# NVIDIA/DeepLearningExamples

Hardware: AMD Instinct MI355X
Metric: training samples/sec (higher is better)
Workload: dtype bf16; 1 GPU; ResNet-50 v1.5 (PyTorch/Classification/ConvNets) synthetic ImageNet 224x224, label smoothing 0.1, SGD momentum 0.875 (BASELINE.json configs[1]); batch_per_gpu=256, global_batch=256, layout=NHWC, hip_graph=False, parallelism=single GPU

## Files before the change

### deeplearningexamples_amd/_cabi.py

```python
import ctypes
import os

import torch

_HERE = os.path.dirname(os.path.abspath(__file__))
LIB_PATH = os.environ.get("DLE_LIB_PATH") or os.path.join(_HERE, "lib", "libdle_mi355x.so")

F32, F16, BF16 = 0, 1, 2
ACT_NONE, ACT_RELU, ACT_GELU, ACT_RELU_BWD, ACT_ADD, ACT_GELU_BWD, ACT_TANH, ACT_TANH_BWD = 0, 1, 2, 3, 4, 5, 6, 7
ACT_ADD_MASKED, ACT_MUL, ACT_GELU_DAUX = 8, 9, 10

_DT = {torch.float32: F32, torch.float16: F16, torch.bfloat16: BF16}

c_void_p, c_int, c_i64, c_float = ctypes.c_void_p, ctypes.c_int, ctypes.c_int64, ctypes.c_float
c_u64 = ctypes.c_uint64

_SIGS = {
    "dle_last_error": (ctypes.c_char_p, []),
    "dle_abi_version": (c_int, []),
    "dle_device_check": (c_int, [c_int, ctypes.c_char_p, c_int]),
    "dle_dot_interact_out_width": (c_int, [c_int, c_int]),
    "dle_dot_interact_fwd": (c_int, [c_void_p, c_void_p, c_int, c_int, c_int, c_int, c_int, c_void_p]),
    "dle_dot_interact_bwd": (c_int, [c_void_p, c_void_p, c_void_p, c_void_p, c_int, c_int, c_int, c_int,
                                     c_int, c_void_p]),
    "dle_dot_interact_bwd_checked": (c_int, [c_void_p, c_void_p, c_void_p, c_void_p, c_int, c_int, c_int, c_int,
                                             c_int, c_void_p, c_void_p]),
    "dle_dlrm_gather_interact_try": (c_int, [c_void_p] * 6 + [c_i64, c_int, c_int, c_int, c_void_p]),
    "dle_emb_gather_fwd": (c_int, [c_void_p, c_void_p, c_void_p, c_void_p, c_void_p, c_i64, c_int, c_int,
                                   c_int, c_i64, c_void_p]),
    "dle_emb_offset_indices": (c_int, [c_void_p, c_void_p, c_void_p, c_void_p, c_i64, c_int, c_void_p]),
    "dle_emb_grad_values": (c_int, [c_void_p, c_void_p, c_void_p, c_i64, c_int, c_void_p]),
    "dle_emb_sparse_sgd": (c_int, [c_void_p, c_void_p, c_void_p, c_void_p, c_float, c_void_p, c_void_p,
                                   c_i64, c_int, c_int, c_i64, c_int, c_void_p]),
    "dle_emb_small_table_mask": (c_int, [c_void_p, c_int, c_int, c_void_p]),
    "dle_emb_sgd_dedup": (c_int, [c_void_p, c_void_p, c_void_p, c_void_p, c_void_p, c_void_p, c_void_p,
                                  c_void_p, c_float, c_void_p, c_void_p, c_i64, c_int, c_int, c_i64, c_int,
                                  c_void_p]),
    "dle_emb_sgd_dedup_ws": (c_int, [c_void_p, c_void_p, c_void_p, c_void_p, c_void_p, c_void_p, c_void_p,
                                     c_void_p, c_float, c_void_p, c_void_p, c_i64, c_int, c_int, c_i64, c_int,
                                     c_void_p, c_i64, c_void_p]),
    "dle_emb_onehot_workspace_bytes": (c_i64, [c_int, c_i64]),
    "dle_emb_sgd_workspace_bytes": (c_i64, [c_void_p, c_int, c_int, c_i64]),
    "dle_emb_onehot_try": (c_int, [c_void_p, c_void_p, c_void_p, c_void_p, c_float, c_void_p, c_void_p, c_void_p, c_void_p,
                                   c_void_p, c_int, c_i64, c_int, c_int, c_i64, c_int, c_void_p, c_i64, c_void_p]),
    "dle_emb_onehot_partials": (c_int, [c_void_p, c_void_p, c_void_p, c_void_p, c_void_p, c_void_p, c_int, c_i64, c_int, c_int,
                                        c_i64, c_int, c_void_p, c_i64, c_void_p, c_void_p]),
    "dle_emb_adam_workspace_bytes": (c_i64, [c_void_p, c_int, c_int, c_i64]),
    "dle_emb_adam_dedup_ws": (c_int, [c_void_p] * 9 + [c_float, c_void_p, c_void_p, c_void_p, c_float, c_float, c_float, c_i64,
                                      c_int, c_int, c_i64, c_int, c_void_p, c_i64, c_void_p]),
    "dle_cast_rows": (c_int, [c_void_p, c_void_p, c_i64, c_int, c_int, c_i64, c_i64, c_int, c_int, c_void_p]),
    "dle_bce_logits": (c_int, [c_void_p, c_void_p, c_void_p, c_void_p, c_void_p, c_i64, c_i64, c_int, c_void_p]),
    "dle_conv1x1_bnbwd_dgrad": (c_int, [c_void_p] * 16 + [c_i64, c_int, c_int, c_int, c_int, c_void_p]),
    "dle_conv1x1_bnbwd_groups": (c_int, [c_int]),
    "dle_conv1x1_bnbwd_dgrad_wgrad": (c_int, [c_void_p] * 15 + [c_i64, c_void_p, c_void_p, c_void_p, c_i64, c_int, c_int, c_int, c_int,
                                              c_void_p]),
    "dle_conv1x1_bnbwd_wgrad_workspace": (c_i64, [c_int, c_int]),
    "dle_gemm_expand_masked_bnred": (c_int, [c_void_p] * 10 + [c_i64, c_int, c_int, c_int, c_i64, c_i64, c_i64, c_int, c_int, c_void_p]),
    "dle_bn_bwd_finish": (c_int, [c_void_p, c_int, c_int, c_void_p, c_void_p, c_int, c_void_p]),
    "dle_gemm_colsum": (c_int, [c_void_p, c_void_p, c_void_p, c_void_p, c_void_p, c_int, c_int, c_int, c_i64, c_i64, c_i64, c_int,
                                c_int, c_int, c_void_p, c_i64, c_void_p]),
    "dle_head_bce_workspace_bytes": (c_i64, [c_i64, c_int]),
    "dle_head_bce_fwd_bwd": (c_int, [c_void_p, c_void_p, c_void_p, c_void_p, c_void_p, c_void_p, c_void_p, c_void_p, c_void_p,
                                     c_void_p, c_void_p, c_void_p, c_i64, c_i64, c_int, c_i64, c_i64, c_int, c_void_p]),
    "dle_amp_update_scale": (c_int, [c_void_p, c_void_p, c_void_p, c_void_p, c_float, c_float, c_int, c_int,
                                     c_void_p]),
    "dle_check_nonfinite": (c_int, [c_void_p, c_void_p, c_i64, c_int, c_void_p]),
    "dle_axpby_f32": (c_int, [c_void_p, c_void_p, c_void_p, c_float, c_float, c_i64, c_void_p]),
    "dle_act_bwd": (c_int, [c_void_p, c_void_p, c_void_p, c_i64, c_int, c_int, c_void_p]),
    "dle_relu_bwd": (c_int, [c_void_p, c_void_p, c_void_p, c_i64, c_int, c_i64, c_i64, c_i64, c_int, c_void_p]),
    "dle_gemm": (c_int, [c_void_p, c_void_p, c_void_p, c_void_p, c_void_p, c_void_p, c_int, c_int, c_int,
                         c_i64, c_i64, c_i64, c_int, c_int, c_int, c_int, c_int, c_int, c_int, c_float,
                         c_void_p, c_i64, c_void_p]),
    "dle_conv2d_fwd": (c_int, [c_void_p, c_void_p, c_void_p, c_void_p] + [c_int] * 12 + [c_void_p]),
    "dle_conv2d_fwd_affine": (c_int, [c_void_p] * 6 + [c_int] * 11 + [c_void_p]),
    "dle_conv3x3_affine_launch_count": (c_i64, []),
    "dle_conv2d_grouped_fwd_affine": (c_int, [c_void_p] * 5 + [c_int] * 9 + [c_void_p]),
    "dle_se_gate": (c_int, [c_void_p] * 6 + [c_int] * 5 + [c_void_p]),
    "dle_se_apply": (c_int, [c_void_p] * 4 + [c_i64, c_int, c_int, c_int, c_int, c_void_p]),
    "dle_dwconv2d_act_fwd": (c_int, [c_void_p] * 6 + [c_i64] + [c_int] * 9 + [c_void_p]),
    "dle_dwconv2d_pool_bands": (c_int, [c_int] * 5),
    "dle_se_gate_act": (c_int, [c_void_p, c_int, c_float] + [c_void_p] * 5 + [c_int] * 4 + [c_void_p]),
    "dle_silu_avgpool_fwd": (c_int, [c_void_p, c_void_p, c_int, c_int, c_int, c_int, c_void_p]),
    "dle_ssd_decode_fwd": (c_int, [c_void_p, c_void_p, c_int, c_void_p, c_void_p, c_void_p, c_int, c_int, c_int, c_float, c_float,
                                   c_int, c_void_p]),
    "dle_ssd_nms_fwd": (c_int, [c_void_p] * 5 + [c_int, c_int, c_int, c_float, c_float, c_int, c_void_p]),
    "dle_ssd_select_fwd": (c_int, [c_void_p] * 9 + [c_int] * 5 + [c_void_p]),
    "dle_conv2d_dgrad": (c_int, [c_void_p, c_void_p, c_void_p, c_void_p] + [c_int] * 10 + [c_void_p]),
    "dle_conv2d_wgrad": (c_int, [c_void_p, c_void_p, c_void_p] + [c_int] * 12 + [c_void_p, c_i64, c_void_p]),
    "dle_nchw_to_nhwc": (c_int, [c_void_p, c_void_p, c_i64, c_int, c_i64, c_int, c_int, c_void_p]),
    "dle_gemm_expand_add_up2": (c_int, [c_void_p, c_void_p, c_void_p, c_void_p, c_int, c_int, c_int, c_i64, c_i64, c_i64, c_i64, c_int,
                                        c_int, c_int, c_int, c_void_p]),
    "dle_conv1x1_bnload_groups": (c_int, [c_int, c_int, c_int]),
    "dle_conv1x1_bnload_fwd": (c_int, [c_void_p] * 11 + [c_i64, c_int, c_int, c_int, c_int, c_void_p]),
    "dle_bn_relu_maxpool_fwd": (c_int, [c_void_p] * 8 + [c_int, c_int, c_int, c_int, c_int, c_void_p]),
    "dle_wgrad1x1_workspace": (c_i64, []),
    "dle_wgrad1x1_mode": (c_int, [c_int]),
    "dle_wgrad1x1_workspace_for": (c_i64, [c_int, c_int, c_int]),
    "dle_gemm8_mode": (c_int, [c_int]),
    "dle_gemm8_min_items": (c_int, [c_int]),
    "dle_gemm8_launch_count": (c_i64, []),
    "dle_wgrad1x1_try": (c_int, [c_void_p, c_void_p, c_void_p, c_int, c_int, c_int, c_int, c_int, c_void_p, c_i64, c_void_p]),
    "dle_conv3x3_wgrad_workspace": (c_i64, []),
    "dle_conv3x3_wgrad_mode": (c_int, [c_int]),
    "dle_stem_conv7_groups": (c_int, [c_int, c_int]),
    "dle_stem_conv7_fwd": (c_int, [c_void_p, c_void_p, c_void_p, c_void_p, c_i64, c_int, c_int, c_int, c_int, c_void_p]),
    "dle_stem_conv7_wgrad_workspace": (c_i64, [c_int, c_int]),
    "dle_stem_conv7_wgrad": (c_int, [c_void_p, c_void_p, c_void_p, c_void_p, c_i64, c_int, c_int, c_int, c_int, c_int, c_void_p]),
    "dle_stem_pack_weight": (c_int, [c_void_p, c_void_p, c_int, c_void_p]),
    "dle_bn_workspace_bytes": (c_i64, [c_i64, c_int]),
    "dle_bn_fwd_stats": (c_int, [c_void_p, c_i64, c_int, c_float, c_float, c_void_p, c_void_p, c_void_p, c_void_p,
                                 c_void_p, c_i64, c_int, c_void_p]),
    "dle_conv2d_fwd_colstats": (c_int, [c_void_p, c_void_p, c_void_p] + [c_int] * 10 + [c_void_p, c_i64, c_void_p, c_void_p]),
    "dle_bn_stats_from_partials": (c_int, [c_void_p, c_int, c_i64, c_int, c_float, c_float, c_void_p, c_void_p, c_void_p,
                                           c_void_p, c_void_p, c_i64, c_void_p]),
    "dle_bn_fwd_apply": (c_int, [c_void_p] * 8 + [c_i64, c_int, c_int, c_int, c_void_p]),
    "dle_rccl_available": (c_int, []),
    "dle_rccl_unique_id": (c_int, [c_void_p]),
    "dle_rccl_init": (c_int, [c_void_p, c_int, c_int, c_void_p]),
    "dle_rccl_count": (c_int, [c_void_p]),
    "dle_rccl_destroy": (c_int, [c_void_p]),
    "dle_rccl_allreduce": (c_int, [c_void_p, c_void_p, c_i64, c_int, c_int, c_void_p]),
    "dle_rccl_broadcast": (c_int, [c_void_p, c_void_p, c_i64, c_int, c_void_p]),
    "dle_rccl_alltoallv": (c_int, [c_void_p, c_void_p, c_void_p, c_void_p, c_void_p, c_int, c_void_p]),
    "dle_gemm8_relu_bits_try": (c_int, [c_void_p] * 5 + [c_int, c_int, c_int, c_i64, c_i64, c_int, c_void_p]),
    "dle_gemm_colsum_bits": (c_int, [c_void_p] * 5 + [c_int, c_int, c_int, c_i64, c_i64, c_int, c_int, c_void_p, c_i64, c_void_p]),
    "dle_bn_bwd_reduce2": (c_int, [c_void_p] * 12 + [c_i64, c_int, c_void_p, c_i64, c_int, c_void_p]),
    "dle_bn_fwd_apply2": (c_int, [c_void_p] * 12 + [c_i64, c_int, c_int, c_void_p]),
    "dle_conv1x1_bnload_fwd2": (c_int, [c_void_p] * 15 + [c_i64, c_int, c_int, c_int, c_int, c_void_p]),
    "dle_bn_bwd_reduce": (c_int, [c_void_p] * 8 + [c_i64, c_int, c_int, c_void_p, c_i64, c_int, c_void_p]),
    "dle_bn_bwd_apply": (c_int, [c_void_p] * 11 + [c_i64, c_int, c_int, c_void_p]),
    "dle_maxpool_fwd": (c_int, [c_void_p, c_void_p, c_void_p] + [c_int] * 8 + [c_void_p]),
    "dle_maxpool_bwd": (c_int, [c_void_p, c_void_p, c_void_p] + [c_int] * 8 + [c_void_p]),
    "dle_pool_bn_bwd_workspace_bytes": (c_i64, [c_int] * 4),
    "dle_pool_bn_bwd": (c_int, [c_void_p] * 10 + [c_int] * 4 + [c_void_p, c_i64, c_int, c_void_p]),
    "dle_avgpool_fwd": (c_int, [c_void_p, c_void_p, c_i64, c_int, c_int, c_int, c_void_p]),
    "dle_avgpool_bwd": (c_int, [c_void_p, c_void_p, c_i64, c_int, c_int, c_int, c_void_p]),
    "dle_upsample_zero": (c_int, [c_void_p, c_void_p, c_i64, c_int, c_int, c_int, c_int, c_int, c_int, c_int, c_void_p]),
    "dle_softmax_xent": (c_int, [c_void_p, c_void_p, c_void_p, c_void_p, c_void_p, c_void_p, c_i64, c_int, c_i64,
                                 c_i64, c_float, c_i64, c_int, c_void_p]),
    "dle_gemm_batched": (c_int, [c_void_p, c_void_p, c_void_p, c_int, c_int, c_int, c_i64, c_i64, c_i64, c_int, c_int,
                                 c_int, c_int, c_float, c_int, c_int, c_i64, c_i64, c_i64, c_i64, c_i64, c_i64, c_void_p]),
    "dle_layernorm_fwd": (c_int, [c_void_p] * 8 + [c_i64, c_int, c_float, c_int, c_void_p]),
    "dle_layernorm_workspace_bytes": (c_i64, [c_int]),
    "dle_layernorm_bwd": (c_int, [c_void_p] * 8 + [c_i64, c_int, c_int, c_void_p, c_i64, c_int, c_void_p]),
    "dle_embed_sum": (c_int, [c_void_p] * 6 + [c_i64, c_int, c_int, c_int, c_void_p]),
    "dle_embed_sum_packed": (c_int, [c_void_p] * 7 + [c_i64, c_int, c_int, c_void_p]),
    "dle_embed_scatter_add": (c_int, [c_void_p, c_void_p, c_void_p, c_i64, c_int, c_int, c_void_p]),
    "dle_rows_select_sum": (c_int, [c_void_p, c_void_p, c_void_p, c_i64, c_int, c_int, c_int, c_void_p, c_i64, c_int,
                                    c_void_p]),
    "dle_rows_gather": (c_int, [c_void_p, c_void_p, c_void_p, c_i64, c_int, c_int, c_void_p]),
    "dle_rows_scatter": (c_int, [c_void_p, c_void_p, c_void_p, c_i64, c_int, c_int, c_int, c_void_p]),
    "dle_softmax_fwd": (c_int, [c_void_p, c_void_p, c_i64, c_int, c_int, c_float, c_int, c_void_p]),
    "dle_softmax_bwd": (c_int, [c_void_p, c_void_p, c_i64, c_int, c_float, c_int, c_void_p]),
    "dle_dropout_add_layernorm_bwd": (c_int, [c_void_p] * 6 + [c_float] + [c_void_p] * 5 + [c_i64, c_int, c_int, c_void_p, c_i64, c_int, c_void_p]),
    "dle_dropout_fwd": (c_int, [c_void_p, c_void_p, c_void_p, c_i64, c_float, c_u64, c_u64, c_void_p, c_int, c_void_p]),
    "dle_dropout_bwd": (c_int, [c_void_p, c_void_p, c_void_p, c_i64, c_float, c_int, c_void_p]),
    "dle_dropout_add_layernorm_fwd": (c_int, [c_void_p] * 9 + [c_i64, c_int, c_float, c_float, c_u64, c_u64, c_void_p, c_int, c_void_p]),
    "dle_softmax_dropout_fwd": (c_int, [c_void_p] * 4 + [c_i64, c_int, c_int, c_float, c_float, c_u64, c_u64, c_void_p, c_int, c_void_p]),
    "dle_softmax_dropout_bwd": (c_int, [c_void_p, c_void_p, c_void_p, c_i64, c_int, c_float, c_float, c_int, c_void_p]),
    "dle_u8_nchw_normalize_nhwc": (c_int, [c_void_p] * 4 + [c_i64, c_int, c_i64, c_int, c_int, c_void_p]),
    "dle_conv2d_dgrad_s2": (c_int, [c_void_p] * 3 + [c_int] * 5 + [c_void_p, c_i64, c_int, c_void_p]),
    "dle_attention_supported": (c_int, [c_int, c_int]),
    "dle_attention_stats_floats": (c_int, [c_int]),
    "dle_attention_fwd": (c_int, [c_void_p] * 5 + [c_int] * 4 + [c_float, c_float, c_u64, c_u64, c_void_p, c_int, c_void_p]),
    "dle_attention_bwd": (c_int, [c_void_p] * 6 + [c_int] * 4 + [c_float, c_float, c_u64, c_u64, c_void_p, c_int, c_void_p]),
    "dle_attention_bwd_keep": (c_int, [c_void_p] * 7 + [c_int] * 4 + [c_float, c_float, c_u64, c_u64, c_void_p, c_int, c_void_p]),
    "dle_attention_varlen_supported": (c_int, [c_int, c_int]),
    "dle_attention_fwd_varlen": (c_int, [c_void_p] * 3 + [c_int, c_int, c_i64, c_int, c_int, c_float, c_int, c_void_p]),
    "dle_attention_varlen_launch_count": (c_u64, []),
    "dle_colsum": (c_int, [c_void_p, c_void_p, c_i64, c_int, c_i64, c_int, c_int, c_void_p, c_i64, c_void_p]),
    "dle_colsum_batched_workspace_bytes": (c_i64, [c_int, c_i64, c_int]),
    "dle_colsum_batched": (c_int, [c_void_p, c_int, c_i64, c_int, c_i64, c_int, c_void_p, c_i64, c_void_p]),
    "dle_mt_table_len": (c_i64, [c_int, c_int]),
    "dle_mt_table_fill": (c_i64, [c_void_p, c_int, c_int, c_void_p, c_void_p, c_int]),
    "dle_mt_l2norm": (c_int, [c_void_p, c_int, c_i64, c_int, c_int, c_void_p, c_void_p, c_void_p, c_int,
                              c_void_p, c_void_p]),
    "dle_mt_lamb_stage1": (c_int, [c_void_p, c_int, c_i64, c_int, c_int, c_void_p, c_float, c_float, c_float,
                                   c_void_p, c_int, c_float, c_int, c_float, c_void_p, c_void_p, c_void_p,
                                   c_void_p]),
    "dle_mt_lamb_stage1_norms": (c_int, [c_void_p, c_int, c_i64, c_int, c_int, c_void_p, c_float, c_float, c_float,
                                         c_void_p, c_int, c_float, c_int, c_float, c_void_p, c_void_p, c_void_p,
                                         c_void_p, c_void_p, c_void_p, c_void_p]),
    "dle_mt_lamb_stage2": (c_int, [c_void_p, c_int, c_i64, c_int, c_int, c_int, c_void_p, c_void_p, c_void_p,
                                   c_void_p, c_float, c_int, c_void_p]),
    "dle_mt_sgd": (c_int, [c_void_p, c_int, c_i64, c_int, c_int, c_int, c_void_p, c_void_p, c_float, c_float,
                           c_float, c_float, c_int, c_int, c_void_p, c_int, c_void_p]),
    "dle_mt_adam": (c_int, [c_void_p, c_int, c_i64, c_int, c_void_p, c_void_p, c_float, c_float, c_float, c_float,
                            c_float, c_void_p, c_void_p, c_void_p, c_float, c_void_p]),
    "dle_mt_adam_copy": (c_int, [c_void_p, c_int, c_i64, c_int, c_int, c_void_p, c_void_p, c_float, c_float, c_float, c_float,
                                 c_void_p, c_void_p, c_void_p, c_void_p]),
    "dle_mt_ema": (c_int, [c_void_p, c_int, c_i64, c_int, c_void_p, c_float, c_float, c_void_p]),
    "dle_wg_taps": (c_int, [c_void_p, c_void_p] + [c_int] * 6 + [c_i64, c_int, c_void_p]),
    "dle_wg_taps_bwd": (c_int, [c_void_p, c_void_p, c_void_p] + [c_int] * 6 + [c_i64, c_i64, c_int, c_void_p]),
    "dle_wg_gate_fwd": (c_int, [c_void_p, c_void_p, c_i64, c_int, c_i64, c_int, c_void_p]),
    "dle_wg_gate_bwd": (c_int, [c_void_p, c_void_p, c_void_p, c_i64, c_int, c_i64, c_i64, c_int, c_void_p]),
    "dle_wg_invconv_fwd": (c_int, [c_void_p, c_void_p, c_void_p, c_void_p, c_i64, c_int, c_int, c_void_p]),
    "dle_wg_invconv_bwd_partials": (c_int, [c_i64]),
    "dle_wg_invconv_bwd": (c_int, [c_void_p] * 8 + [c_float, c_void_p, c_i64, c_int, c_void_p]),
    "dle_wg_logdet_inv": (c_int, [c_void_p, c_void_p, c_void_p, c_void_p, c_int, c_void_p]),
    "dle_wg_coupling_partials": (c_int, [c_i64]),
    "dle_wg_coupling_fwd": (c_int, [c_void_p, c_void_p, c_void_p, c_void_p, c_i64, c_int, c_void_p]),
    "dle_wg_coupling_bwd": (c_int, [c_void_p] * 6 + [c_float, c_i64, c_int, c_int, c_void_p]),
    "dle_wg_loss": (c_int, [c_void_p, c_void_p, c_int, c_void_p, c_int, c_float, c_i64, c_void_p, c_void_p, c_void_p]),
    "dle_wg_dz_init": (c_int, [c_void_p, c_void_p, c_void_p, c_float, c_i64, c_void_p]),
    "dle_wg_weight_norm_fwd": (c_int, [c_void_p, c_void_p, c_void_p] + [c_int] * 5 + [c_void_p]),
    "dle_wg_weight_norm_bwd": (c_int, [c_void_p] * 5 + [c_int] * 4 + [c_void_p]),
    "dle_wg_upsample_weight": (c_int, [c_void_p] * 4 + [c_int] * 4 + [c_void_p]),
    "dle_wg_upsample_weight_bwd": (c_int, [c_void_p, c_void_p, c_int, c_int, c_int, c_void_p]),
    "dle_wg_weight_norm_fwd_batched": (c_int, [c_void_p, c_int, c_i64, c_int, c_void_p]),
    "dle_wg_weight_norm_bwd_batched": (c_int, [c_void_p, c_int, c_i64, c_void_p]),
    "dle_wg_logdet_inv_batched": (c_int, [c_void_p, c_void_p, c_void_p, c_void_p, c_void_p, c_int, c_void_p]),
    "dle_wg_flow_inv": (c_int, [c_void_p] * 6 + [c_i64, c_int, c_int, c_int, c_float, c_int, c_int, c_void_p]),
    "dle_wg_flow_inv_first": (c_int, [c_void_p, c_void_p, c_void_p, c_i64, c_int, c_float, c_int, c_void_p]),
    "dle_t2_tanh_fwd": (c_int, [c_void_p, c_void_p, c_i64, c_int, c_void_p]),
    "dle_t2_lstm_fwd": (c_int, [c_void_p, c_i64, c_void_p, c_void_p, c_void_p, c_i64, c_void_p, c_i64, c_void_p, c_i64, c_void_p,
                                c_i64, c_float, c_void_p, c_void_p, c_i64, c_void_p, c_i64, c_int, c_int, c_int, c_void_p]),
    "dle_t2_lstm_bwd": (c_int, [c_void_p, c_i64, c_void_p, c_i64, c_void_p, c_i64, c_void_p, c_void_p, c_i64, c_void_p, c_void_p,
                                c_i64, c_void_p, c_void_p, c_i64, c_float, c_void_p, c_void_p, c_int, c_int, c_int, c_void_p]),
    "dle_t2_attention_fwd": (c_int, [c_void_p] * 10 + [c_i64, c_void_p, c_i64, c_void_p, c_i64, c_void_p] + [c_int] * 7 + [c_void_p]),
    "dle_t2_attention_bwd": (c_int, [c_void_p, c_i64, c_void_p, c_i64, c_void_p, c_i64] + [c_void_p] * 14 + [c_int, c_int, c_void_p, c_void_p] +
                             [c_int] * 5 + [c_void_p]),
    "dle_a2a_blocks": (c_int, [c_void_p, c_void_p, c_int, c_int, c_void_p, c_int, c_int, c_void_p]),
    "dle_t2_sum_steps": (c_int, [c_void_p, c_void_p, c_int, c_i64, c_int, c_void_p]),
    "dle_t2_location_bwd": (c_int, [c_void_p, c_void_p, c_void_p, c_int, c_int, c_int, c_int, c_void_p]),
    "dle_transpose_cast": (c_int, [c_void_p, c_void_p, c_int, c_int, c_i64, c_i64, c_int, c_int, c_void_p]),
    "dle_t2_mel_loss": (c_int, [c_void_p, c_i64, c_void_p, c_void_p, c_void_p, c_void_p, c_i64, c_void_p, c_void_p, c_void_p, c_i64,
                                c_int, c_int, c_void_p]),
    "dle_t2_lstm_gemm_fwd": (c_int, [c_void_p, c_i64, c_void_p, c_i64, c_void_p, c_void_p, c_void_p, c_void_p, c_void_p, c_i64, c_void_p,
                                     c_i64, c_void_p, c_i64, c_void_p, c_i64, c_void_p, c_i64, c_float, c_int, c_int, c_int, c_int,
                                     c_void_p]),
    "dle_t2_mask_rows": (c_int, [c_void_p, c_i64, c_int, c_void_p, c_i64, c_int, c_float, c_int, c_void_p]),
    "dle_t2_prenet_infer": (c_int, [c_void_p, c_void_p, c_void_p, c_void_p, c_i64, c_void_p, c_void_p, c_u64, c_void_p, c_int, c_int,
                                    c_int, c_int, c_void_p]),
    "dle_t2_frame_infer": (c_int, [c_void_p, c_i64, c_void_p, c_i64] + [c_void_p] * 7 + [c_int, c_float, c_int, c_i64, c_void_p,
                                   c_void_p, c_void_p, c_i64, c_u64, c_int, c_int, c_int, c_int, c_int, c_void_p]),
    "dle_conv1d_lrelu_fwd": (c_int, [c_void_p] * 6 + [c_int] * 6 + [c_float, c_float, c_int, c_void_p]),
    "dle_hfg_post_fwd": (c_int, [c_void_p] * 4 + [c_int] * 4 + [c_float, c_int, c_void_p]),
    "dle_conv1d_packed_fwd": (c_int, [c_void_p] * 6 + [c_int, c_int, c_i64, c_int, c_int, c_int, c_float, c_int, c_void_p]),
    "dle_fp_relu_layernorm_fwd": (c_int, [c_void_p] * 7 + [c_i64, c_int, c_int, c_float, c_int, c_void_p]),
    "dle_fp_embed": (c_int, [c_void_p] * 6 + [c_int, c_int, c_i64, c_int, c_int, c_int, c_int, c_void_p]),
    "dle_fp_scalar_conv_add": (c_int, [c_void_p] * 5 + [c_int, c_int, c_i64, c_int, c_int, c_int, c_void_p]),
    "dle_fp_durations": (c_int, [c_void_p, c_int] + [c_void_p] * 5 + [c_int, c_int, c_i64, c_float, c_float, c_int, c_void_p]),
    "dle_fp_expand": (c_int, [c_void_p] * 7 + [c_int, c_int, c_i64, c_int, c_i64, c_int, c_int, c_int, c_void_p]),
    "dle_fp_unpack_mel": (c_int, [c_void_p] * 4 + [c_int, c_i64, c_int, c_int, c_int, c_void_p]),
# ... 183 lines not shown
```

### deeplearningexamples_amd/convnets/engine.py

```python
import copy
import math
from typing import Optional

import numpy as np
import os

import torch
import torch.distributed as dist

from .. import functional as F
from .. import multi_tensor as mt
from ..utils.amp import GradScalerState
from ..utils.buckets import GradBuckets
from ..utils import comm
from .resnet import Deferred, ResNet50


def lr_cosine_policy(base_lr, warmup_length, epochs, end_lr=0.0):
    def fn(iteration, epoch):
        if epoch < warmup_length:
            return base_lr * (epoch + 1) / warmup_length
        e, es = epoch - warmup_length, epochs - warmup_length
        return end_lr + 0.5 * (1 + np.cos(np.pi * e / es)) * (base_lr - end_lr)
    return fn


def lr_step_policy(base_lr, steps, decay_factor, warmup_length):
    def fn(iteration, epoch):
        if epoch < warmup_length:
            return base_lr * (epoch + 1) / warmup_length
        lr = base_lr
        for s in steps:
            if epoch >= s:
                lr *= decay_factor
        return lr
    return fn


def lr_linear_policy(base_lr, warmup_length, epochs):
    def fn(iteration, epoch):
        if epoch < warmup_length:
            return base_lr * (epoch + 1) / warmup_length
        return base_lr * (1 - (epoch - warmup_length) / (epochs - warmup_length))
    return fn


class ResNetTrainer:
    def __init__(self, model: ResNet50, lr: float, momentum=0.875, weight_decay=3.0517578125e-05, nesterov=False,
                 label_smoothing=0.1, compute_dtype=torch.bfloat16, bn_weight_decay=False, static_loss_scale=1.0,
                 world_size=1, process_group=None, bucket_mb=25, grad_acc_steps=1, ema=None):
        self.model = model
        self.grad_acc_steps = max(1, int(grad_acc_steps))
        self.steps_since_update = 0
        self.flat_acc = None
        self.dev = model.fc.weight.device
        self.dtype = compute_dtype
        self.momentum, self.wd, self.nesterov, self.smoothing = momentum, weight_decay, nesterov, label_smoothing
        self.world, self.pg = world_size, process_group
        self.bn_weight_decay = bn_weight_decay
        if world_size > 1:
            comm.broadcast_parameters_(list(model.parameters()) + list(model.buffers()), 0, process_group)
        self.stem, self.blocks = model.units()
        self.scaler = GradScalerState(self.dev, enabled=compute_dtype == torch.float16, init_scale=static_loss_scale,
                                      growth_interval=int(1e9))
        self.lr = torch.full((1,), lr, dtype=torch.float32, device=self.dev)
        self.first_step = True
        self.steps_done = 0
        named = dict(model.named_parameters())
        order = ["fc.weight", "fc.bias"]
        for (u1, u2, u3, ud) in reversed(self.blocks):
            for u in ([u3, ud] if ud is not None else [u3]) + [u2, u1]:
                order += [u.name_conv + ".weight", u.name_bn + ".weight", u.name_bn + ".bias"]
        order += ["conv1.weight", "bn1.weight", "bn1.bias"]
        assert sorted(order) == sorted(named), "parameter bookkeeping out of sync with the module tree"
        self.names = order
        self.params = [named[n] for n in order]
        total = sum(p.numel() for p in self.params)
        self.flat_grad = torch.zeros(total, dtype=torch.float32, device=self.dev)
        self.flat_mom = torch.zeros(total, dtype=torch.float32, device=self.dev)
        self.gview, self.mview, self.offset = {}, {}, {}
        o = 0
        for n, p in zip(order, self.params):
            self.offset[n] = o
            self.gview[n] = self.flat_grad[o:o + p.numel()]
            self.mview[n] = self.flat_mom[o:o + p.numel()]
            o += p.numel()
        self.comm_stream = torch.cuda.Stream(device=self.dev) if world_size > 1 else None
        self.buckets = GradBuckets(self.flat_grad, [(n, p.numel()) for n, p in zip(order, self.params)], bucket_mb,
                                   process_group, self.comm_stream) if world_size > 1 else None
        self.w16 = {}
        units = [self.stem] + [u for blk in self.blocks for u in blk if u is not None]
        self.units = units
        for u in units:
            w = named[u.name_conv + ".weight"]
            ko, ci, r, s = w.shape
            cp = (ci + 7) // 8 * 8
            u.w16 = torch.zeros((ko, r, s, cp), dtype=compute_dtype, device=self.dev)
            self.w16[u.name_conv + ".weight"] = u.w16
            u.ggamma = self.gview[u.name_bn + ".weight"]
            u.gbeta = self.gview[u.name_bn + ".bias"]
            if cp == ci:
                u.gw = self.gview[u.name_conv + ".weight"].view(ko, r, s, ci)
            else:
                u.gw = torch.zeros((ko, r, s, cp), dtype=torch.float32, device=self.dev)
        self.wgrad_stream = torch.cuda.Stream(device=self.dev) if (self.dev.type == "cuda" and
                                                                   os.environ.get("DLE_RN50_WGRAD_STREAM", "1") != "0") else None
        self._wgrad_keepalive = []
        for u in units:
            u.wgrad_stream, u.keepalive = self.wgrad_stream, self._wgrad_keepalive
        self.branch_stream = torch.cuda.Stream(device=self.dev) if (self.dev.type == "cuda" and
                                                                    os.environ.get("DLE_RN50_BRANCH_STREAM", "1") != "0") else None
        self._branch_keep = []
        if self.buckets is not None:
            self.buckets.extra_streams += [st for st in (self.wgrad_stream, self.branch_stream) if st is not None]
        self.stem4 = os.environ.get("DLE_RN50_STEM4", "1") != "0"
        self.fuse_up2 = os.environ.get("DLE_RN50_FUSE_UP2", "1") != "0"
        self.fuse_bn = os.environ.get("DLE_RN50_FUSE_BN", "1") != "0"
        self.fuse_bnred = os.environ.get("DLE_RN50_FUSE_BNRED", "1") != "0"
        self.fuse_dsbn = os.environ.get("DLE_RN50_FUSE_DSBN", "1") != "0"
        self.fuse_dsred = os.environ.get("DLE_RN50_FUSE_DSRED", "1") != "0"
        self.fuse_pool_bwd = os.environ.get("DLE_RN50_FUSE_POOLBWD", "1") != "0"
        self.stem.w2 = torch.zeros((64, 7, 8, 4), dtype=compute_dtype, device=self.dev)
        self.stem.gw_flat = self.gview["conv1.weight"]
        self.fc_w16 = torch.empty(model.fc.weight.shape, dtype=compute_dtype, device=self.dev)
        self.w16["fc.weight"] = self.fc_w16
        self.refresh_working_copies()
        self._build_tables()
        self.ema = None if ema is None else float(ema)
        self.ema_model = None
        if self.ema is not None:
            self._build_ema()

    @staticmethod
    def _phys(p):
        if p.dim() == 4:
            return p.data.permute(0, 2, 3, 1).reshape(-1)
        return p.data.reshape(-1)

    def _refresh_copies(self, model, units, stem, fc_w16):
        for u in units:
            w = u.conv.weight
            ko, ci, r, s = w.shape
            F.cast_rows(self._phys(w).view(ko * r * s, ci), self.dtype, cols_out=u.w16.shape[-1],
                        out=u.w16.view(ko * r * s, -1))
        F.cast(model.fc.weight.data, self.dtype, out=fc_w16)
        F.stem_pack_weight(model.conv1.weight.data, self.dtype, out=stem.w2)

    def refresh_working_copies(self):
        self._refresh_copies(self.model, self.units, self.stem, self.fc_w16)

    def _stem_image(self, images):
        cp = 4 if (self.stem4 and images.shape[-1] <= 224) else 8
        if images.dtype == torch.uint8:
            if getattr(self, "_mean_std", None) is None:
                from .dataloaders import IMAGENET_MEAN, IMAGENET_STD
                self._mean_std = (torch.tensor(IMAGENET_MEAN, device=self.dev) * 255.0, torch.tensor(IMAGENET_STD, device=self.dev) * 255.0)
            return F.u8_nchw_normalize_nhwc(images, self._mean_std[0], self._mean_std[1], self.dtype, cp)
        return F.nchw_to_nhwc(images, self.dtype, cp)

    def _build_tables(self):
        named = dict(zip(self.names, self.params))
        decay_copy, decay_plain, nodecay = ([], [], [], []), ([], [], []), ([], [], [])
        for n, p in named.items():
            g, m, ph = self.gview[n], self.mview[n], self._phys(p)
            assert ph.data_ptr() == p.data_ptr(), "parameter %s is not dense in memory order" % n
            if "bn" in n and not self.bn_weight_decay:
                for lst, t in zip(nodecay, (g, ph, m)):
                    lst.append(t)
            elif n in self.w16 and self.w16[n].numel() == p.numel():
                for lst, t in zip(decay_copy, (g, ph, m, self.w16[n].view(-1))):
                    lst.append(t)
            else:
                for lst, t in zip(decay_plain, (g, ph, m)):
                    lst.append(t)
        self.t_decay_copy = mt.TensorTable(list(decay_copy))
        self.t_decay_plain = mt.TensorTable(list(decay_plain))
        self.t_nodecay = mt.TensorTable(list(nodecay))

    def set_lr(self, lr: float):
        self.lr.fill_(lr)

    @staticmethod
    def _ema_entries(model):
        return [(k, v) for k, v in model.state_dict().items() if not k.endswith("num_batches_tracked")]

    def _build_ema(self):
        self.ema_model = copy.deepcopy(self.model)
        xs, es = [], []
        for (k, x), (ke, e) in zip(self._ema_entries(self.model), self._ema_entries(self.ema_model)):
            assert k == ke and x.shape == e.shape and x.stride() == e.stride(), "EMA copy of %s lost the master's layout" % k
            assert x.dtype == torch.float32 and e.dtype == torch.float32, "EMA runs on the fp32 master state (%s)" % k
            px, pe = self._phys(x), self._phys(e)
            assert px.data_ptr() == x.data_ptr() and pe.data_ptr() == e.data_ptr(), "%s is not dense in memory order" % k
            xs.append(px)
            es.append(pe)
        self.t_ema = mt.TensorTable([xs, es], chunk=mt.streaming_chunk([xs]))
        self.ema_coef = torch.empty(2, dtype=torch.float32, device=self.dev)
        self._ema_coef_views = (self.ema_coef[0:1], self.ema_coef[1:2])
        self._ema_mu_t = None
        self.set_ema_step(None)
        self.ema_stem, self.ema_blocks = self.ema_model.units()
        self.ema_units = [self.ema_stem] + [u for blk in self.ema_blocks for u in blk if u is not None]
        for u, src in zip(self.ema_units, self.units):
            u.w16 = torch.zeros_like(src.w16)
        self.ema_stem.w2 = torch.zeros_like(self.stem.w2)
        self.ema_fc_w16 = torch.empty_like(self.fc_w16)
        self.ema_dirty = True

    def set_ema_step(self, step):
        if self.ema is None:
            raise ValueError("this trainer keeps no averaged model: construct it with ema=<decay>")
        mu_t = self.ema if step is None else min(self.ema, (1.0 + step) / (10 + step))
        if mu_t != self._ema_mu_t:
            self._ema_coef_views[0].fill_(mu_t)
            self._ema_coef_views[1].fill_(1.0 - mu_t)
            self._ema_mu_t = mu_t
        self.ema_dirty = True

    def mark_ema_dirty(self):
        self.ema_dirty = True

    def _ema_eval_state(self):
        if self.ema is None:
            raise ValueError("this trainer keeps no averaged model: construct it with ema=<decay>")
        if self.ema_dirty:
            self._refresh_copies(self.ema_model, self.ema_units, self.ema_stem, self.ema_fc_w16)
            self.ema_dirty = False
        return self.ema_model, self.ema_stem, self.ema_blocks, self.ema_fc_w16

    def set_side_streams(self, enabled):
        if not hasattr(self, "_streams_saved"):
            self._streams_saved = (self.wgrad_stream, self.branch_stream)
        torch.cuda.synchronize(self.dev)
        self.wgrad_stream, self.branch_stream = self._streams_saved if enabled else (None, None)
        for u in self.units:
            u.wgrad_stream = self.wgrad_stream

    def _maybe_reduce(self, finished_param_name):
        if self.buckets is not None and getattr(self, "_reduce_now", True):
            self.buckets.grad_ready(finished_param_name)

    def _input(self, images):
        if images.dim() == 4 and not images.is_contiguous():
            images = images.contiguous()
        return images

    def infer(self, images, ema=False):
        model, stem, blocks, fc_w16 = self._ema_eval_state() if ema else (self.model, self.stem, self.blocks, self.fc_w16)
        x = self._stem_image(self._input(images))
        h, _ = F.maxpool_fwd(stem.forward_eval(x))
        for (u1, u2, u3, ud) in blocks:
            res = ud.forward_eval(h) if ud is not None else h
            h = u3.forward_eval(u2.forward_eval(u1.forward_eval(h)), residual=res)
        pooled = F.avgpool_fwd(h)
        return F.gemm(pooled, fc_w16, pooled.shape[0], fc_w16.shape[0], fc_w16.shape[1], True, True,
                      out_dtype=torch.float32, bias=model.fc.bias.data)

    def eval_step(self, images, target, ema=False):
        logits = self.infer(images, ema=ema)
        loss, _ = F.softmax_xent(logits, target, smoothing=0.0)
        return loss, logits

    def forward(self, images):
        x = self._stem_image(self._input(images))
        d0 = self.stem.forward(x, defer=self.fuse_bn)
        if isinstance(d0, Deferred) and d0.t.shape[1] % 2 == 0 and d0.t.shape[2] % 2 == 0:
            m0, self._amax, mask0 = F.bn_relu_maxpool_fwd(d0.t, d0.mean, d0.rstd, self.stem.bn.weight.data, self.stem.bn.bias.data)
            d0._done(None, mask0)
            self._pool_in_hw = d0.t.shape[1:3]
        else:
            a0 = d0.materialize() if isinstance(d0, Deferred) else d0
            m0, self._amax = F.maxpool_fwd(a0)
            self._pool_in_hw = a0.shape[1:3]
        h = m0
        bs = self.branch_stream
        fuse = self.fuse_bn
        for (u1, u2, u3, ud) in self.blocks:
            o1 = u1.forward(h)
            hy = h.y if isinstance(h, Deferred) else h
            if ud is not None and bs is not None:
                cur = torch.cuda.current_stream()
                bs.wait_stream(cur)
                self._branch_keep.clear()
                with torch.cuda.stream(bs):
                    res = ud.forward(hy, defer=self.fuse_dsbn)
                o2 = u2.forward(o1, defer=fuse)
                cur.wait_stream(bs)
                self._branch_keep.append(res)
            else:
                res = ud.forward(hy, defer=self.fuse_dsbn) if ud is not None else hy
                o2 = u2.forward(o1, defer=fuse)
            h = u3.forward(o2, residual=res, defer=fuse)
        if isinstance(h, Deferred):
            h = h.materialize()
        self._feat_hw = h.shape[1:3]
        self._pooled = F.avgpool_fwd(h)
        n = self._pooled.shape[0]
        logits = F.gemm(self._pooled, self.fc_w16, n, self.fc_w16.shape[0], self.fc_w16.shape[1], True, True,
                        out_dtype=torch.float32, bias=self.model.fc.bias.data)
        return logits

    def backward(self, dlogits):
        n = dlogits.shape[0]
        fcw = self.fc_w16
        if self.buckets is not None:
            self.buckets.fired = 0
        F.gemm(dlogits, self._pooled, fcw.shape[0], fcw.shape[1], n, False, False,
               out=self.gview["fc.weight"].view(fcw.shape), splitk=F.pick_splitk(fcw.shape[0], fcw.shape[1], n))
        F.colsum(dlogits, out=self.gview["fc.bias"])
        self._maybe_reduce("fc.weight"); self._maybe_reduce("fc.bias")
        gp = F.gemm(dlogits, fcw, n, fcw.shape[1], fcw.shape[0], True, False)
        g = F.avgpool_bwd(gp, self._feat_hw)
        for blk in self.blocks:
            for u in blk:
                if u is not None:
                    u.reduce_done = False
        for bi in range(len(self.blocks) - 1, -1, -1):
            u1, u2, u3, ud = self.blocks[bi]
            mask3 = u3.relu_mask()
            if ud is not None and self.fuse_dsred and u3.saved is not None and ud.saved is not None and mask3 is not None \
                    and not u3.reduce_done and u3.saved[1].shape == ud.saved[1].shape:
                F.bn_bwd_reduce2(g, mask3, u3.saved[1], u3.saved[3], u3.saved[4], u3.ggamma, u3.gbeta,
                                 ud.saved[1], ud.saved[3], ud.saved[4], ud.ggamma, ud.gbeta)
                u3.reduce_done = ud.reduce_done = True
            bs = self.branch_stream if ud is not None else None
            if bs is not None:
                cur = torch.cuda.current_stream()
                bs.wait_stream(cur)
                self._branch_keep.clear()
                with torch.cuda.stream(bs):
                    gskip = ud.backward(g, dy_mask=mask3, compact_dx=self.fuse_up2)
                self._branch_keep.append((gskip, g))
            g3 = u3.backward(g, bnred=u2 if self.fuse_bnred else None)
            self._done(u3)
            if ud is not None and bs is None:
                gskip = ud.backward(g, dy_mask=mask3, compact_dx=self.fuse_up2)
            elif ud is None:
                gskip = (g, mask3)
            g2 = u2.backward(g3)
            self._done(u2)
            if bs is not None:
                cur.wait_stream(bs)
            if ud is not None:
                self._done(ud)
            prev3 = self.blocks[bi - 1][2] if (self.fuse_bnred and ud is None and bi > 0) else None
            g = u1.backward(g2, dx_addend=gskip, bnred=prev3)
            self._done(u1)
        if self.fuse_pool_bwd:
            self.stem.backward(None, need_dx=False, pooled=(g, self._amax))
        else:
            g = F.maxpool_bwd(g, self._amax, self._pool_in_hw)
            self.stem.backward(g, need_dx=False)
        gw = self.stem.gw
        ko, r, s, cp = gw.shape
        stem_generic = self.stem.saved_c != 4
        if self.wgrad_stream is not None:
            torch.cuda.current_stream().wait_stream(self.wgrad_stream)
            self._wgrad_keepalive.clear()
        self._branch_keep.clear()
        if stem_generic:
            F.copy_rows(gw.view(ko * r * s, cp)[:, :3], self.gview["conv1.weight"].view(ko * r * s, 3))
        self._done(self.stem)

    def _done(self, u):
        for suffix, nm in ((".weight", u.name_conv), (".weight", u.name_bn), (".bias", u.name_bn)):
            self._maybe_reduce(nm + suffix)

    def optimizer_step(self):
        sc = self.scaler
        skip = sc.found_inf if sc.enabled else None
        inv = sc.inv_scale if sc.enabled else None
        kw = dict(momentum=self.momentum, nesterov=self.nesterov, first_step=self.first_step, skip_flag=skip,
                  inv_scale=inv, has_momentum=self.momentum != 0)
        mt.sgd(self.t_decay_copy, self.lr, weight_decay=self.wd, model_copy=True, **kw)
        mt.sgd(self.t_decay_plain, self.lr, weight_decay=self.wd, **kw)
        mt.sgd(self.t_nodecay, self.lr, weight_decay=0.0, **kw)
        u = self.stem
        w = self.model.conv1.weight
        F.stem_pack_weight(w.data, self.dtype, out=u.w2)
        ko, ci, r, s = w.shape
        F.cast_rows(self._phys(w).view(ko * r * s, ci), self.dtype, cols_out=u.w16.shape[-1], out=u.w16.view(ko * r * s, -1))
        self.first_step = False

    def train_step(self, images, target, step=None):
        loss = self._train_step(images, target)
        if self.ema is not None:
            if step is not None:
                self.set_ema_step(step)
            mt.ema(self.t_ema, self.ema, coef=self.ema_coef)
            self.ema_dirty = True
        return loss

    def _train_step(self, images, target):
        sc = self.scaler
        acc = self.grad_acc_steps
        self.steps_since_update += 1
        last = self.steps_since_update == acc
        logits = self.forward(images)
        gs = sc.scale if sc.enabled else None
        if isinstance(target, tuple):
            ya, yb, lam = target
            la, da = F.softmax_xent(logits, ya, smoothing=self.smoothing, grad_scale=gs, grad_dtype=torch.float32)
            lb, db = F.softmax_xent(logits, yb, smoothing=self.smoothing, grad_scale=gs, grad_dtype=torch.float32)
            loss = lam * la + (1.0 - lam) * lb
            F.axpby_(da.view(-1), db.view(-1), da.view(-1), lam, 1.0 - lam)
            dlogits = F.cast(da, self.dtype)
        else:
            loss, dlogits = F.softmax_xent(logits, target, smoothing=self.smoothing, grad_scale=gs, grad_dtype=self.dtype)
        self._reduce_now = acc == 1
        self.backward(dlogits)
        if acc > 1:
            if self.flat_acc is None:
                self.flat_acc = torch.empty_like(self.flat_grad)
            first = self.steps_since_update == 1
            dst = self.flat_grad if last else self.flat_acc
            F.axpby_(self.flat_grad, None if first else self.flat_acc, dst, 1.0 / acc, 0.0 if first else 1.0)
            loss = loss / acc
            if not last:
                self.steps_done += 1
                return loss
            if self.world > 1:
                comm.allreduce_mean_(self.flat_grad, self.pg)
        elif self.buckets is not None:
            self.buckets.wait()
        if sc.enabled:
            F.check_nonfinite_(self.flat_grad, sc.found_inf)
        self.optimizer_step()
        sc.update()
        self.steps_since_update = 0
        self.steps_done += 1
        return loss

    def reduced_loss(self, loss):
        if self.world > 1:
            loss = comm.allreduce_mean_(loss.clone(), self.pg)
        return loss

    def sync_counters(self):
        for u in self.units:
            u.bn.num_batches_tracked.fill_(self.steps_done)
```

### deeplearningexamples_amd/convnets/resnet.py

```python
from contextlib import nullcontext as _nullcontext
from typing import List

import os

import torch
from torch import nn

from .. import _cabi as C
from .. import functional as F

LAYERS, WIDTHS, EXPANSION = [3, 4, 6, 3], [64, 128, 256, 512], 4


def _conv(cin, cout, k, stride, device):
    m = nn.Conv2d(cin, cout, kernel_size=k, stride=stride, padding=(k - 1) // 2, bias=False, device=device)
    nn.init.kaiming_normal_(m.weight, mode="fan_in", nonlinearity="relu")
    m.weight.data = m.weight.data.contiguous(memory_format=torch.channels_last)
    return m


def _bn(c, device, zero_init=False):
    m = nn.BatchNorm2d(c, device=device)
    nn.init.constant_(m.weight, 0 if zero_init else 1)
    nn.init.constant_(m.bias, 0)
# ... 10 lines not shown
        r = self.residual
        if isinstance(r, Deferred):
            return r.t, (r.mean, r.rstd, r.unit.bn.weight.data, r.unit.bn.bias.data)
        return r, None

    def _done(self, y, mask):
        u = self.unit
        u.saved = (u.saved[0], self.t, mask, self.mean, self.rstd)
        self.y = y

    def materialize(self):
        if self.y is None:
            u = self.unit
            res, res_bn = self.residual_args()
            y, mask = F.bn_fwd_apply(self.t, self.mean, self.rstd, u.bn.weight.data, u.bn.bias.data, residual=res,
                                     relu=u.relu, want_mask=True, residual_bn=res_bn)
            self._done(y, mask)
        return self.y


class ConvBN:

    def __init__(self, conv: nn.Conv2d, bn: nn.BatchNorm2d, name_conv: str, name_bn: str, relu: bool):
        self.conv, self.bn, self.name_conv, self.name_bn, self.relu = conv, bn, name_conv, name_bn, relu
        self.k = conv.kernel_size[0]
        self.stride, self.pad = conv.stride[0], conv.padding[0]
        self.cin, self.cout = conv.in_channels, conv.out_channels
        self.w16 = None
        self.gw = self.ggamma = self.gbeta = None
        self.saved = None
        self.w2 = self.gw_flat = None
        self.wgrad_stream = None
        self.fuse_bnbwd = os.environ.get("DLE_RN50_FUSE_BNBWD", "1") != "0"
        self.fuse_bnbwd_wgrad = os.environ.get("DLE_RN50_FUSE_BNBWD_WGRAD", "1") != "0"
        self.reduce_done = False
        self.keepalive = None

    def forward(self, x, residual=None, defer=False):
        t = None
        if isinstance(x, Deferred):
            d, r = x, None
            if self.k == 1 and self.stride == 1 and d.unit.relu and d.y is None:
                res, res_bn = d.residual_args()
                r = F.conv1x1_bnload_fwd(d.t, res, self.w16, d.mean, d.rstd, d.unit.bn.weight.data, d.unit.bn.bias.data,
                                         self.bn.running_mean, self.bn.running_var, eps=self.bn.eps, momentum=self.bn.momentum,
                                         res_bn=res_bn)
            if r is not None:
                t, x, bits, mean, rstd = r
                d._done(x, bits)
            else:
                x = d.materialize()
        if t is None:
            if x.shape[-1] == 4:
                t, mean, rstd = F.stem_conv_fwd_bnstats(x, self.w2, self.bn.running_mean, self.bn.running_var, eps=self.bn.eps,
                                                        momentum=self.bn.momentum)
            else:
                t, mean, rstd = F.conv2d_fwd_bnstats(x, self.w16, self.stride, self.pad, self.bn.running_mean,
                                                     self.bn.running_var, eps=self.bn.eps, momentum=self.bn.momentum)
        if defer:
            self.saved = (x, t, None, mean, rstd)
            return Deferred(self, t, mean, rstd, residual)
        if isinstance(residual, Deferred):
            d = Deferred(self, t, mean, rstd, residual)
            self.saved = (x, t, None, mean, rstd)
            return d.materialize()
        y, mask = F.bn_fwd_apply(t, mean, rstd, self.bn.weight.data, self.bn.bias.data, residual=residual,
                                 relu=self.relu, want_mask=True)
        self.saved = (x, t, mask, mean, rstd)
        return y

    def forward_eval(self, x, residual=None):
        t = F.stem_conv_fwd(x, self.w2, want_stats=False)[0] if x.shape[-1] == 4 else F.conv2d_fwd(x, self.w16, self.stride, self.pad)
        rstd = torch.rsqrt(self.bn.running_var + self.bn.eps)
        y, _ = F.bn_fwd_apply(t, self.bn.running_mean, rstd, self.bn.weight.data, self.bn.bias.data, residual=residual,
                              relu=self.relu, want_mask=False)
        return y

    def backward(self, dy, need_dx=True, dx_addend=None, dy_mask=None, compact_dx=False, bnred=None, pooled=None):
        x, t, mask, mean, rstd = self.saved
        self.saved = None
        self.saved_c = x.shape[-1]
        rmask = mask if self.relu else dy_mask
        n, h, w, c = x.shape
        reduce_done, self.reduce_done = self.reduce_done, False
        fused = None
        wgrad_done = False
        if self.fuse_bnbwd and self.k == 1 and self.stride == 1 and need_dx and dx_addend is None:
            b2 = None
            if bnred is not None and bnred.saved is not None and bnred.relu:
                b2 = (bnred.saved[1], bnred.saved[2], bnred.saved[3], bnred.saved[4], bnred.ggamma, bnred.gbeta)
            if self.fuse_bnbwd_wgrad and pooled is None and self.gw is not None:
                r = F.bn_bwd_conv1x1_dgrad_wgrad(dy, t, mean, rstd, self.bn.weight.data, self.ggamma, self.gbeta,
                                                 self.w16.view(self.cout, c), x, self.gw, relu_mask=rmask,
                                                 reduce_done=reduce_done, bnred=b2)
                if r is not None:
                    fused, wgrad_done = (None, r[0], r[1]), True
            if fused is None:
                fused = F.bn_bwd_conv1x1_dgrad(dy, t, mean, rstd, self.bn.weight.data, self.ggamma, self.gbeta,
                                               self.w16.view(self.cout, c), relu_mask=rmask, reduce_done=reduce_done, bnred=b2)
        gt = None
        if pooled is not None:
            if self.relu and not reduce_done:
                gt = F.pool_bn_bwd(pooled[0], pooled[1], t, mean, rstd, self.bn.weight.data, self.ggamma, self.gbeta, rmask)
            if gt is None:
                dy = F.maxpool_bwd(pooled[0], pooled[1], t.shape[1:3])
        if gt is not None:
            pass
        elif fused is not None:
            gt = fused[0]
            if fused[2]:
                bnred.reduce_done = True
        else:
            gt, _ = F.bn_bwd(dy, None, t, mean, rstd, self.bn.weight.data, self.ggamma, self.gbeta, relu_mask=rmask,
                             reduce_done=reduce_done)
        up2 = isinstance(dx_addend, tuple) and dx_addend[0] == "up2"
        masked = isinstance(dx_addend, tuple) and not up2
        ws = self.wgrad_stream if not wgrad_done else None
        if ws is not None:
            ws.wait_stream(torch.cuda.current_stream())
            self.keepalive.append((gt, x))
        with (torch.cuda.stream(ws) if ws is not None else _nullcontext()):
            if wgrad_done:
                pass
            elif c == 4:
                F.stem_conv_wgrad(gt, x, self.gw_flat)
            elif self.k == 1 and self.stride == 1:
                m = n * h * w
                if not F.wgrad1x1(gt.view(m, self.cout), x.view(m, c), self.gw.view(self.cout, c)):
                    F.gemm(gt.view(m, self.cout), x.view(m, c), self.cout, c, m, False, False, out=self.gw.view(self.cout, c),
                           splitk=F.pick_splitk(self.cout, c, m, target_blocks=1024))
            else:
                F.conv2d_wgrad(gt, x, (self.k, self.k), self.stride, self.pad, out=self.gw)
        dx = None
        if fused is not None:
            dx = fused[1].view(n, h, w, c)
        elif self.k == 1 and self.stride == 1:
            m = n * h * w
            g2 = gt.view(m, self.cout)
            if need_dx:
                if masked:
                    dxf = None
                    if bnred is not None and bnred.saved is not None and bnred.relu:
                        _, pt, pmask, pmean, prstd = bnred.saved
                        dxf = F.gemm_masked_add_bnred(g2, self.w16.view(self.cout, c), m, c, self.cout, dx_addend[0].view(m, c),
                                                      dx_addend[1], pt.view(m, c), pmask, pmean, prstd, bnred.ggamma,
                                                      bnred.gbeta) if pt.numel() == m * c else None
                        if dxf is not None:
                            bnred.reduce_done = True
                    dx = (dxf if dxf is not None else
                          F.gemm(g2, self.w16.view(self.cout, c), m, c, self.cout, True, False, act=C.ACT_ADD_MASKED,
                                 mask_src=dx_addend[0].view(m, c), aux=dx_addend[1])).view(n, h, w, c)
                else:
                    if up2:
                        dx = F.gemm_add_upsampled2(g2, self.w16.view(self.cout, c), dx_addend[1], dx_addend[2])
                        if dx is not None:
                            return dx.view(n, h, w, c)
                        dx_addend = F.upsample_zero(dx_addend[1], dx_addend[2], 2)
                    dx = F.gemm(g2, self.w16.view(self.cout, c), m, c, self.cout, True, False,
                                act=C.ACT_ADD if dx_addend is not None else C.ACT_NONE,
                                mask_src=dx_addend.view(m, c) if dx_addend is not None else None).view(n, h, w, c)
        else:
            assert not masked and not up2, "masked / compact residual gradients enter through the 1x1 convolution of a bottleneck"
            if need_dx and compact_dx and self.k == 1 and self.stride == 2 and dx_addend is None and h % 2 == 0 and w % 2 == 0:
                dx = ("up2", F.conv1x1_s2_dgrad_compact(gt, self.w16), (h, w))
            else:
                dx = F.conv2d_dgrad(gt, self.w16, (h, w), self.stride, self.pad, addend=dx_addend) if need_dx else None
        return dx

    def relu_mask(self):
        return self.saved[2]


class Bottleneck(nn.Module):
    def __init__(self, inplanes, planes, stride, downsample, device, last_bn_0_init=False):
        super().__init__()
        self.conv1 = _conv(inplanes, planes, 1, 1, device)
        self.bn1 = _bn(planes, device)
        self.conv2 = _conv(planes, planes, 3, stride, device)
        self.bn2 = _bn(planes, device)
        self.conv3 = _conv(planes, planes * EXPANSION, 1, 1, device)
        self.bn3 = _bn(planes * EXPANSION, device, zero_init=last_bn_0_init)
        self.relu = nn.ReLU(inplace=True)
        self.downsample = downsample
        self.stride = stride


class ResNet50(nn.Module):
    def __init__(self, num_classes=1000, last_bn_0_init=False, device="cuda"):
        super().__init__()
        self.conv1 = _conv(3, 64, 7, 2, device)
        self.bn1 = _bn(64, device)
        self.relu = nn.ReLU(inplace=True)
        self.maxpool = nn.MaxPool2d(kernel_size=3, stride=2, padding=1)
        inplanes = 64
        layers = []
        for i, (w, n) in enumerate(zip(WIDTHS, LAYERS)):
            blocks = []
            for b in range(n):
                stride = (1 if i == 0 else 2) if b == 0 else 1
                down = None
                if b == 0:
                    down = nn.Sequential(_conv(inplanes, w * EXPANSION, 1, stride, device), _bn(w * EXPANSION, device))
                blocks.append(Bottleneck(inplanes, w, stride, down, device, last_bn_0_init))
                inplanes = w * EXPANSION
            layers.append(nn.Sequential(*blocks))
        self.layers = nn.Sequential(*layers)
        self.avgpool = nn.AdaptiveAvgPool2d(1)
        self.fc = nn.Linear(512 * EXPANSION, num_classes, device=device)

    def units(self) -> List:
        stem = ConvBN(self.conv1, self.bn1, "conv1", "bn1", relu=True)
        blocks = []
        for li, layer in enumerate(self.layers):
            for bi, blk in enumerate(layer):
                pre = "layers.%d.%d." % (li, bi)
                u1 = ConvBN(blk.conv1, blk.bn1, pre + "conv1", pre + "bn1", True)
                u2 = ConvBN(blk.conv2, blk.bn2, pre + "conv2", pre + "bn2", True)
                u3 = ConvBN(blk.conv3, blk.bn3, pre + "conv3", pre + "bn3", True)
                ud = None
                if blk.downsample is not None:
                    ud = ConvBN(blk.downsample[0], blk.downsample[1], pre + "downsample.0", pre + "downsample.1", False)
                blocks.append((u1, u2, u3, ud))
        return stem, blocks
```

### deeplearningexamples_amd/csrc/gemm_expand.hip

```cpp
#include "gemm_tiles.h"

#define EX_TN 128
#define EX_PAD 8

struct ExpandArgs {
  const unsigned short* A;
  const unsigned short* B;
  unsigned short* C;
  const unsigned short* src;
  const unsigned char* bits;
  float* stats;
  int M, N, K;
  long long lda, ldb, ldc;
  int b_kc, row_tiles, groups, col_tiles;
  FastDiv dHW, dW;
  int up_HW, up_W, up_P, up_Q;
  long long ld_src;
  const unsigned short* t2;
  const unsigned char* bits2;
  const float* mean2;
  const float* rstd2;
};

template <int DT> struct ExMfma;
template <> struct ExMfma<DLE_F16> {
  static __device__ __forceinline__ float4_t run(ushort8_t a, ushort8_t b, float4_t c) {
    return __builtin_amdgcn_mfma_f32_16x16x32_f16(__builtin_bit_cast(half8_t, a), __builtin_bit_cast(half8_t, b), c, 0, 0, 0);
  }
};
template <> struct ExMfma<DLE_BF16> {
  static __device__ __forceinline__ float4_t run(ushort8_t a, ushort8_t b, float4_t c) {
    return __builtin_amdgcn_mfma_f32_16x16x32_bf16(__builtin_bit_cast(bf16x8_t, a), __builtin_bit_cast(bf16x8_t, b), c, 0, 0, 0);
  }
};

__device__ __forceinline__ int ex_pos(int nl) {
  const int j = nl >> 5, r = nl & 31;
  return 32 * j + 16 * ((r >> 2) & 1) + 4 * (r >> 3) + (r & 3);
}

template <int KS, int ACT, bool BRED = false>
struct ExStream {
  ushort8_t fa[KS];
  ushort8_t sv[ACT ? 4 : 1];
  ushort8_t tv[BRED ? 4 : 1];
  uint4_t mb;
  uint4_t mb2;
  long long o0;
  bool live;
  bool has;
  __device__ __forceinline__ void load_a(const ExpandArgs& p, int m, int kg) {
    const long long mr = m < p.M ? m : p.M - 1;
    const unsigned short* arow = p.A + mr * p.lda + kg * 8;
#pragma unroll
    for (int ks = 0; ks < KS; ++ks) fa[ks] = *(const ushort8_t*)(arow + ks * 32);
  }
  __device__ __forceinline__ void load_src(const ExpandArgs& p, int m, int n0, int kg) {
    live = m < p.M;
    const long long mr = live ? m : p.M - 1;
    o0 = mr * p.ldc + n0 + kg * 8;
    if (ACT == 3) {
      const int mi = (int)mr;
      const int n = fd_div(mi, p.dHW), rem = mi - n * p.up_HW;
      const int h = fd_div(rem, p.dW), w = rem - h * p.up_W;
      has = !((h | w) & 1);
      const long long cr = has ? ((long long)n * p.up_P + (h >> 1)) * p.up_Q + (w >> 1) : 0;
      const unsigned short* srow = p.src + cr * p.ld_src + n0 + kg * 8;
#pragma unroll
      for (int j = 0; j < 4; ++j) sv[j] = *(const ushort8_t*)(srow + 32 * j);
    } else if (ACT) {
#pragma unroll
      for (int j = 0; j < 4; ++j) sv[j] = *(const ushort8_t*)(p.src + o0 + 32 * j);
    }
    if (ACT == 2) mb = *(const uint4_t*)(p.bits + ((mr * p.ldc + n0) >> 3));
    if (BRED) {
#pragma unroll
      for (int j = 0; j < 4; ++j) tv[j] = *(const ushort8_t*)(p.t2 + o0 + 32 * j);
      mb2 = *(const uint4_t*)(p.bits2 + ((mr * p.ldc + n0) >> 3));
    }
  }
};

__device__ __forceinline__ void ex_reduce_scatter16(const float* v, int fr, float* acc) {
  float w16[16], w8[8], w4[4];
  const bool h8 = fr & 8, h4 = fr & 4, h2 = fr & 2, h1 = fr & 1;
#pragma unroll
  for (int q = 0; q < 16; ++q) {
    const float keep = h8 ? v[16 + q] : v[q], send = h8 ? v[q] : v[16 + q];
    w16[q] = keep + __shfl_xor(send, 8, 64);
  }
#pragma unroll
  for (int q = 0; q < 8; ++q) {
    const float keep = h4 ? w16[8 + q] : w16[q], send = h4 ? w16[q] : w16[8 + q];
    w8[q] = keep + __shfl_xor(send, 4, 64);
  }
#pragma unroll
  for (int q = 0; q < 4; ++q) {
    const float keep = h2 ? w8[4 + q] : w8[q], send = h2 ? w8[q] : w8[4 + q];
    w4[q] = keep + __shfl_xor(send, 2, 64);
  }
#pragma unroll
  for (int q = 0; q < 2; ++q) {
    const float keep = h1 ? w4[2 + q] : w4[q], send = h1 ? w4[q] : w4[2 + q];
    acc[q] += keep + __shfl_xor(send, 1, 64);
  }
}

template <int DT, int KS, int ACT, bool STATS, int NW, bool BRED = false>
__global__ __launch_bounds__(NW * 64) __attribute__((amdgpu_waves_per_eu((STATS || BRED) ? 3 : 4)))
void gemm_expand_kernel(ExpandArgs p) {
  constexpr int K = KS * 32, LDW = K + EX_PAD, TM = NW * 16;
  extern __shared__ __attribute__((aligned(16))) unsigned char smem_raw[];
  unsigned short* wl = (unsigned short*)smem_raw;
  const int lane = threadIdx.x & 63, wave = threadIdx.x >> 6;
  const int fr = lane & 15, kg = lane >> 4;
  const int xcd = blockIdx.x & 7, slot = blockIdx.x >> 3;
  const int tn = slot % p.col_tiles, g = (slot / p.col_tiles) * 8 + xcd;
  const int n0 = tn * EX_TN;
  if (p.b_kc) {
    constexpr int CPR = K / 8;
    for (int c = threadIdx.x; c < EX_TN * CPR; c += NW * 64) {
      const int nl = c / CPR, kc = c - nl * CPR;
      const ushort8_t v = *(const ushort8_t*)(p.B + (long long)(n0 + nl) * p.ldb + kc * 8);
      *(ushort8_t*)(wl + ex_pos(nl) * LDW + kc * 8) = v;
    }
  } else {
    for (int c = threadIdx.x; c < K * (EX_TN / 8); c += NW * 64) {
      const int k = c >> 4, nc = c & 15;
      const ushort8_t v = *(const ushort8_t*)(p.B + (long long)k * p.ldb + n0 + nc * 8);
#pragma unroll
      for (int e = 0; e < 8; ++e) wl[ex_pos(nc * 8 + e) * LDW + k] = v[e];
    }
  }
  float* mu2 = (float*)(smem_raw + EX_TN * LDW * 2);
  if (BRED) {
    for (int c = threadIdx.x; c < EX_TN; c += NW * 64) { mu2[c] = p.mean2[n0 + c]; mu2[EX_TN + c] = p.rstd2[n0 + c]; }
  }
  __syncthreads();
  float s1[STATS ? 32 : 1], s2[STATS ? 32 : 1];
  if (STATS) {
#pragma unroll
    for (int i = 0; i < 32; ++i) { s1[i] = 0.f; s2[i] = 0.f; }
  }
  float b1[2] = {0.f, 0.f}, b2s[2] = {0.f, 0.f};
  const unsigned short* wrow = wl + fr * LDW + kg * 8;
  const int mrow = wave * 16 + fr;
  ExStream<KS, ACT, BRED> cur;
  cur.load_a(p, g * TM + mrow, kg);
  cur.load_src(p, g * TM + mrow, n0, kg);
  for (int tm = g; tm < p.row_tiles; tm += p.groups) {
    const int m_next = (tm + p.groups) * TM + mrow;
    float4_t acc[8];
#pragma unroll
    for (int b = 0; b < 8; ++b) acc[b] = (float4_t){0.f, 0.f, 0.f, 0.f};
#pragma unroll
    for (int ks = 0; ks < KS; ++ks) {
#pragma unroll
      for (int b = 0; b < 8; ++b) {
        const ushort8_t fw = *(const ushort8_t*)(wrow + b * 16 * LDW + ks * 32);
        acc[b] = ExMfma<DT>::run(fw, cur.fa[ks], acc[b]);
      }
      __builtin_amdgcn_sched_barrier(0);
    }
    cur.load_a(p, m_next, kg);
    ushort8_t outv[4];
    float tg[BRED ? 32 : 1], tx[BRED ? 32 : 1];
    const bool live_cur = cur.live;
    const bool has_cur = ACT == 3 ? cur.has : true;
#pragma unroll
    for (int j = 0; j < 4; ++j) {
      float v[8];
#pragma unroll
      for (int r = 0; r < 4; ++r) { v[r] = acc[2 * j][r]; v[4 + r] = acc[2 * j + 1][r]; }
      if (ACT) {
        float y[8];
        unpack8<DT>(cur.sv[j], y);
        const unsigned int bits8 = ACT == 2 ? (cur.mb[j] >> (8 * kg)) & 0xffu : 0xffu;
#pragma unroll
        for (int r = 0; r < 8; ++r) {
          if (ACT == 2) { if ((bits8 >> r) & 1u) v[r] += y[r]; }
          else if (ACT == 3) { if (has_cur) v[r] += y[r]; }
          else v[r] += y[r];
        }
      }
      const ushort8_t ov = pack8<DT>(v);
      outv[j] = ov;
      if (STATS) {
        float z[8];
        unpack8<DT>(ov, z);
#pragma unroll
        for (int r = 0; r < 8; ++r) {
          const float zz = live_cur ? z[r] : 0.f;
          s1[8 * j + r] += zz;
          s2[8 * j + r] += zz * zz;
        }
      }
      if (BRED) {
        float z[8], tf[8];
        unpack8<DT>(ov, z);
        unpack8<DT>(cur.tv[j], tf);
        const unsigned b2 = (cur.mb2[j] >> (8 * kg)) & 0xffu;
        const float4_t m0 = *(const float4_t*)(mu2 + 32 * j + 8 * kg), m1 = *(const float4_t*)(mu2 + 32 * j + 8 * kg + 4);
        const float4_t r0 = *(const float4_t*)(mu2 + EX_TN + 32 * j + 8 * kg), r1 = *(const float4_t*)(mu2 + EX_TN + 32 * j + 8 * kg + 4);
#pragma unroll
        for (int r = 0; r < 8; ++r) {
          const float gz = (live_cur && ((b2 >> r) & 1u)) ? z[r] : 0.f;
          const float mu = r < 4 ? m0[r & 3] : m1[r & 3], rs = r < 4 ? r0[r & 3] : r1[r & 3];
          tg[8 * j + r] = gz;
          tx[8 * j + r] = gz * (tf[r] - mu) * rs;
        }
      }
    }
    if (BRED) {
      ex_reduce_scatter16(tg, fr, b1);
      ex_reduce_scatter16(tx, fr, b2s);
    }
    __builtin_amdgcn_sched_barrier(0);
    cur.load_src(p, m_next, n0, kg);
    __builtin_amdgcn_sched_barrier(0);
    {
      const bool odd = fr & 1;
      const int m_cur = tm * TM + mrow;
      const bool live_other = (odd ? m_cur - 1 : m_cur + 1) < p.M;
      const long long o_own = (long long)m_cur * p.ldc + n0 + kg * 8;
      const long long o_other = odd ? o_own - p.ldc : o_own + p.ldc;
#pragma unroll
      for (int h = 0; h < 2; ++h) {
        const uint4_t mine0 = __builtin_bit_cast(uint4_t, outv[2 * h]), mine1 = __builtin_bit_cast(uint4_t, outv[2 * h + 1]);
        const uint4_t give = odd ? mine0 : mine1;
        uint4_t got;
#pragma unroll
        for (int q = 0; q < 4; ++q) got[q] = (unsigned)__shfl_xor((int)give[q], 1, 64);
        const uint4_t first = odd ? got : mine0, second = odd ? mine1 : got;
        const long long o_first = (odd ? o_other : o_own) + 64 * h + (odd ? 32 : 0);
        const long long o_second = (odd ? o_own : o_other) + 64 * h + (odd ? 32 : 0);
        const bool live_first = odd ? live_other : live_cur, live_second = odd ? live_cur : live_other;
        if (live_first) *(uint4_t*)(p.C + o_first) = first;
        if (live_second) *(uint4_t*)(p.C + o_second) = second;
      }
    }
  }
  if (BRED) {
    __syncthreads();
    float* red = (float*)smem_raw;
#pragma unroll
    for (int b = 0; b < 2; ++b) {
      const int i = 2 * fr + b, col = 32 * (i >> 3) + 8 * kg + (i & 7);
      red[(wave * 2 + 0) * EX_TN + col] = b1[b];
      red[(wave * 2 + 1) * EX_TN + col] = b2s[b];
    }
    __syncthreads();
    for (int t = threadIdx.x; t < 2 * EX_TN; t += NW * 64) {
      const int which = t / EX_TN, col = t - which * EX_TN;
      float tot = 0.f;
#pragma unroll
      for (int w = 0; w < NW; ++w) tot += red[(w * 2 + which) * EX_TN + col];
      p.stats[((long long)g * 2 + which) * p.N + n0 + col] = tot;
    }
  }
  if (STATS) {
#pragma unroll
    for (int i = 0; i < 32; ++i) {
#pragma unroll
      for (int o = 1; o < 16; o <<= 1) {
        s1[i] += __shfl_xor(s1[i], o, 64);
        s2[i] += __shfl_xor(s2[i], o, 64);
      }
    }
    __syncthreads();
    float* red = (float*)smem_raw;
    if (fr == 0) {
#pragma unroll
      for (int i = 0; i < 32; ++i) {
        const int col = 32 * (i >> 3) + 8 * kg + (i & 7);
        red[(wave * 2 + 0) * EX_TN + col] = s1[i];
        red[(wave * 2 + 1) * EX_TN + col] = s2[i];
      }
    }
    __syncthreads();
    for (int t = threadIdx.x; t < 2 * EX_TN; t += NW * 64) {
      const int which = t / EX_TN, col = t - which * EX_TN;
      float tot = 0.f;
#pragma unroll
      for (int w = 0; w < NW; ++w) tot += red[(w * 2 + which) * EX_TN + col];
      p.stats[((long long)g * 2 + which) * p.N + n0 + col] = tot;
    }
  }
}

static int ex_rows_per_tile(int K) { return K > 128 ? 128 : 64; }
extern "C" int dle_gemm_expand_groups(int M, int N, int K) {
  const int tm = ex_rows_per_tile(K), row_tiles = (M + tm - 1) / tm, col_tiles = N / EX_TN;
  const int per_cu = K > 128 ? 2 : 4;
  const int resident = 256 * per_cu;
  int groups = (resident + col_tiles - 1) / (col_tiles > 0 ? col_tiles : 1);
  if (groups > row_tiles) groups = row_tiles;
  return (groups + 7) / 8 * 8;
}

extern "C" int dle_gemm_expand_try(const void* A, const void* B, void* C, const void* src, const void* bits, float* stats, int M,
                                   int N, int K, int64_t lda, int64_t ldb, int64_t ldc, int b_kc, int in_dtype, int out_dtype,
                                   int act, hipStream_t stream) {
  if (M < 4096 || (K != 64 && K != 128 && K != 256) || (N % EX_TN) != 0 || N < 2 * K || out_dtype != in_dtype) return 0;
  if (((((uintptr_t)A) | ((uintptr_t)B) | ((uintptr_t)C) | ((uintptr_t)src)) & 15) != 0 || (lda & 7) || (ldb & 7) || (ldc & 7)) return 0;
  if (act < EX_ACT_NONE || act > EX_ACT_ADD_MASKED) return 0;
  if (act == EX_ACT_ADD_MASKED && !bits) return 0;
  if (act == EX_ACT_ADD_MASKED && ((ldc % EX_TN) != 0 || (((uintptr_t)bits) & 15) != 0)) return 0;
  if (act && !src) return 0;
  ExpandArgs p = {(const unsigned short*)A, (const unsigned short*)B, (unsigned short*)C, (const unsigned short*)src,
                  (const unsigned char*)bits, stats, M, N, K, (long long)lda, (long long)ldb, (long long)ldc, b_kc, 0, 0, 0};
  const int tmr = ex_rows_per_tile(K);
  p.row_tiles = (M + tmr - 1) / tmr;
  p.col_tiles = N / EX_TN;
  p.groups = dle_gemm_expand_groups(M, N, K);
  const int lds_bytes = EX_TN * (K + EX_PAD) * 2 > 8 * 2 * EX_TN * 4 ? EX_TN * (K + EX_PAD) * 2 : 8 * 2 * EX_TN * 4;
  const dim3 grid((unsigned)(p.groups * p.col_tiles)), block(tmr * 4);
#define GO(DT, KS, ACT, ST)                                                                                              \
  do {                                                                                                                   \
    constexpr int NW_ = KS > 4 ? 8 : 4;                                                                                  \
    DLE_LAUNCH_LDS((gemm_expand_kernel<DT, KS, ACT, ST, NW_>), grid, block, lds_bytes, stream, p);                       \
  } while (0)
#define PICK_ACT(DT, KS)                                              \
  do {                                                                \
    if (stats) { if (act != EX_ACT_NONE) return 0; GO(DT, KS, EX_ACT_NONE, true); } \
    else if (act == EX_ACT_NONE) GO(DT, KS, EX_ACT_NONE, false);                    \
    else if (act == EX_ACT_ADD) GO(DT, KS, EX_ACT_ADD, false);                      \
    else GO(DT, KS, EX_ACT_ADD_MASKED, false);                                      \
  } while (0)
#define PICK_K(DT)                                   \
  do {                                               \
    if (K == 64) PICK_ACT(DT, 2);                    \
    else if (K == 128) PICK_ACT(DT, 4);              \
    else PICK_ACT(DT, 8);                            \
  } while (0)
  if (in_dtype == DLE_F16) PICK_K(DLE_F16); else PICK_K(DLE_BF16);
#undef PICK_K
#undef PICK_ACT
#undef GO
  hipError_t e = hipGetLastError();
  if (e != hipSuccess) { dle_set_error("gemm_expand launch failed: %s", hipGetErrorString(e)); return (int)e + 1000; }
  return 1;
}

extern "C" int dle_gemm_expand_masked_bnred(const void* A, const void* B, void* C, const void* src, const void* bits, const void* t2,
                                            const void* bits2, const float* mean2, const float* rstd2, float* partial,
                                            int64_t partial_bytes, int M, int N, int K, int64_t lda, int64_t ldb, int64_t ldc,
                                            int b_kc, int dtype, hipStream_t stream) {
  if (!dle_gemm_expand_enabled()) return 0;
  const int k256 = dle_env_int("DLE_GEMM_BNRED_K256", 0);
  if (M < 4096 || (K != 64 && K != 128 && !(K == 256 && k256)) || (N % EX_TN) != 0 || N < 2 * K) return 0;
  if (dtype != DLE_F16 && dtype != DLE_BF16) return 0;
  if (!A || !B || !C || !src || !bits || !t2 || !bits2 || !mean2 || !rstd2 || !partial) return 0;
  if (((((uintptr_t)A) | ((uintptr_t)B) | ((uintptr_t)C) | ((uintptr_t)src) | ((uintptr_t)t2) | ((uintptr_t)bits) | ((uintptr_t)bits2)) & 15) != 0 ||
      (lda & 7) || (ldb & 7) || (ldc % EX_TN) != 0)
    return 0;
  ExpandArgs p = {(const unsigned short*)A, (const unsigned short*)B, (unsigned short*)C, (const unsigned short*)src,
                  (const unsigned char*)bits, partial, M, N, K, (long long)lda, (long long)ldb, (long long)ldc, b_kc, 0, 0, 0};
  p.t2 = (const unsigned short*)t2; p.bits2 = (const unsigned char*)bits2; p.mean2 = mean2; p.rstd2 = rstd2;
  const int tmr = ex_rows_per_tile(K);
  p.row_tiles = (M + tmr - 1) / tmr;
  p.col_tiles = N / EX_TN;
  p.groups = dle_gemm_expand_groups(M, N, K);
  if (partial_bytes < (long long)p.groups * 2 * N * 4) return 0;
  size_t lds_bytes = (size_t)EX_TN * (K + EX_PAD) * 2 + 2 * EX_TN * 4;
  if (lds_bytes < (size_t)8 * 2 * EX_TN * 4) lds_bytes = (size_t)8 * 2 * EX_TN * 4;
  const dim3 grid((unsigned)(p.groups * p.col_tiles)), block(tmr * 4);
#define GO(DT, KS)                                                                                                       \
  do {                                                                                                                   \
    constexpr int NW_ = KS > 4 ? 8 : 4;                                                                                  \
    DLE_LAUNCH_LDS((gemm_expand_kernel<DT, KS, 2, false, NW_, true>), grid, block, lds_bytes, stream, p);                \
  } while (0)
#define PICK_K(DT) do { if (K == 64) GO(DT, 2); else if (K == 128) GO(DT, 4); else GO(DT, 8); } while (0)
  if (dtype == DLE_F16) PICK_K(DLE_F16); else PICK_K(DLE_BF16);
#undef PICK_K
#undef GO
  hipError_t e = hipGetLastError();
  if (e != hipSuccess) { dle_set_error("gemm_expand_masked_bnred launch failed: %s", hipGetErrorString(e)); return (int)e + 1000; }
  return 1;
}

extern "C" int dle_gemm_expand_add_up2(const void* A, const void* B, void* C, const void* compact, int M, int N, int K, int64_t lda,
                                       int64_t ldb, int64_t ldc, int64_t ld_compact, int b_kc, int H, int W, int dtype,
                                       hipStream_t stream) {
  if (M < 4096 || (K != 64 && K != 128 && K != 256) || (N % EX_TN) != 0 || N < 2 * K) return 0;
  if (dtype != DLE_F16 && dtype != DLE_BF16) return 0;
  if ((H & 1) || (W & 1) || H <= 0 || W <= 0 || (M % (H * W)) != 0 || !compact) return 0;
  if (((((uintptr_t)A) | ((uintptr_t)B) | ((uintptr_t)C) | ((uintptr_t)compact)) & 15) != 0 || (lda & 7) || (ldb & 7) || (ldc & 7) ||
      (ld_compact & 7)) return 0;
  if (!dle_gemm_expand_enabled()) return 0;
  ExpandArgs p = {(const unsigned short*)A, (const unsigned short*)B, (unsigned short*)C, (const unsigned short*)compact, nullptr,
                  nullptr, M, N, K, (long long)lda, (long long)ldb, (long long)ldc, b_kc, 0, 0, 0};
  p.dHW = make_fastdiv(H * W); p.dW = make_fastdiv(W);
  p.up_HW = H * W; p.up_W = W; p.up_P = H / 2; p.up_Q = W / 2; p.ld_src = ld_compact;
  const int tmr = ex_rows_per_tile(K);
  p.row_tiles = (M + tmr - 1) / tmr;
  p.col_tiles = N / EX_TN;
  p.groups = dle_gemm_expand_groups(M, N, K);
  const int lds_bytes = EX_TN * (K + EX_PAD) * 2;
  const dim3 grid((unsigned)(p.groups * p.col_tiles)), block(tmr * 4);
#define GO3(DT, KS)                                                                                                      \
  do {                                                                                                                   \
    constexpr int NW_ = KS > 4 ? 8 : 4;                                                                                  \
    DLE_LAUNCH_LDS((gemm_expand_kernel<DT, KS, 3, false, NW_>), grid, block, lds_bytes, stream, p);                      \
  } while (0)
#define PICK3(DT) do { if (K == 64) GO3(DT, 2); else if (K == 128) GO3(DT, 4); else GO3(DT, 8); } while (0)
  if (dtype == DLE_F16) PICK3(DLE_F16); else PICK3(DLE_BF16);
#undef PICK3
#undef GO3
  hipError_t e = hipGetLastError();
  if (e != hipSuccess) { dle_set_error("gemm_expand_add_up2 launch failed: %s", hipGetErrorString(e)); return (int)e + 1000; }
  return 1;
}
```

### deeplearningexamples_amd/functional.py

```python
import ctypes
import os

import torch

from . import _cabi as C


def dot_interact_out_width(rows, cols):
    return C.lib().dle_dot_interact_out_width(rows, cols)


def dot_interact_fwd(x, force_generic=False):
    C.require_cuda(x)
    if x.dim() != 3:
        raise ValueError("dot_interact: expected [batch, rows, cols], got %s" % (tuple(x.shape),))
    x = x.contiguous()
    b, r, c = x.shape
    out = torch.empty((b, dot_interact_out_width(r, c)), dtype=x.dtype, device=x.device)
    C.annotate(bytes=float(b) * (r * c + out.shape[1]) * x.element_size())
    C.call("dle_dot_interact_fwd", C.ptr(x), C.ptr(out), b, r, c, C.dt(x), int(force_generic), C.stream())
    return out


def dot_interact_bwd(x, upstream, force_generic=False, fuse_mlp_grad=False, grad_out=None, found_inf=None):
# ... 736 lines not shown
    name = "ssd_decode"
    if not 1 <= len(heads) <= SSD_MAX_MAPS or len(geom) != len(heads):
        raise ValueError("%s: 1..%d feature maps with one (nd, loc, conf) each" % (name, SSD_MAX_MAPS))
    h0 = heads[0]
    if h0.dtype not in _FP16:
        raise ValueError("%s: 16-bit head outputs only (got %s)" % (name, h0.dtype))
    n, table, b = h0.shape[0], [], 0
    for t, (nd, loc, conf) in zip(heads, geom):
        if t.dim() != 4 or t.shape[0] != n or t.shape[1] != t.shape[2] or t.dtype != h0.dtype or not t.is_contiguous():
            raise ValueError("%s: every head must be a contiguous [N, fs, fs, pitch] tensor of one dtype" % name)
        table += [int(t.shape[1]), int(nd), int(t.shape[3]), int(loc), int(conf)]
        b += int(nd) * int(t.shape[1]) ** 2
    if dboxes_xywh.dtype != torch.float32 or tuple(dboxes_xywh.shape) != (b, 4) or not dboxes_xywh.is_contiguous():
        raise ValueError("%s: dboxes_xywh must be a contiguous fp32 [B,4] = [%d,4] tensor" % (name, b))
    C.require_cuda(dboxes_xywh, *heads)
    boxes = torch.empty((n, b, 4), dtype=torch.float32, device=h0.device)
    probs = torch.empty((n, int(num_labels), b), dtype=torch.float32, device=h0.device)
    ptrs = (ctypes.c_void_p * len(heads))(*[t.data_ptr() for t in heads])
    g = (ctypes.c_int * len(table))(*table)
    C.call("dle_ssd_decode_fwd", ptrs, g, len(heads), C.ptr(dboxes_xywh), C.ptr(boxes), C.ptr(probs), n, b, int(num_labels),
           float(scale_xy), float(scale_wh), C.dt(h0), C.stream())
    return boxes, probs


def _ssd_boxes_probs(name, boxes, probs):
    if boxes.dim() != 3 or boxes.shape[2] != 4 or boxes.dtype != torch.float32 or not boxes.is_contiguous():
        raise ValueError("%s: boxes must be a contiguous fp32 [N,B,4] tensor" % name)
    if probs is not None and (probs.dim() != 3 or probs.dtype != torch.float32 or not probs.is_contiguous()
                              or probs.shape[0] != boxes.shape[0] or probs.shape[2] != boxes.shape[1]):
        raise ValueError("%s: probs must be a contiguous fp32 [N,L,B] tensor" % name)


def ssd_nms(boxes, probs, criteria=0.5, threshold=0.05, max_num=200):
    name = "ssd_nms"
    _ssd_boxes_probs(name, boxes, probs)
    n, l, b = probs.shape
    C.require_cuda(boxes, probs)
    max_num = int(max_num)
    m = max(max_num, 1)
    kept_idx = torch.empty((n, max(l - 1, 0), m), dtype=torch.int32, device=boxes.device)
    kept_score = torch.empty((n, max(l - 1, 0), m), dtype=torch.float32, device=boxes.device)
    kept_count = torch.empty((n, max(l - 1, 0)), dtype=torch.int32, device=boxes.device)
    C.call("dle_ssd_nms_fwd", C.ptr(boxes), C.ptr(probs), C.ptr(kept_idx), C.ptr(kept_score), C.ptr(kept_count), n, b, l,
           float(threshold), float(criteria), max_num, C.stream())
    return kept_idx, kept_score, kept_count


def ssd_select(boxes, kept_idx, kept_score, kept_count, max_output=200):
    name = "ssd_select"
    _ssd_boxes_probs(name, boxes, None)
    n, b = boxes.shape[:2]
    if (kept_idx.dim() != 3 or kept_idx.dtype != torch.int32 or kept_score.dtype != torch.float32 or kept_idx.shape != kept_score.shape
            or kept_count.dtype != torch.int32 or tuple(kept_count.shape) != tuple(kept_idx.shape[:2]) or kept_idx.shape[0] != n
            or not (kept_idx.is_contiguous() and kept_score.is_contiguous() and kept_count.is_contiguous())):
        raise ValueError("%s: kept_idx int32 / kept_score fp32 [N,L-1,max_num] and kept_count int32 [N,L-1], contiguous (ssd_nms)" % name)
    C.require_cuda(boxes, kept_idx, kept_score, kept_count)
    lm1, max_num = kept_idx.shape[1:]
    max_output = int(max_output)
    m = max(max_output, 1)
    dev = boxes.device
    det_boxes = torch.empty((n, m, 4), dtype=torch.float32, device=dev)
    det_label = torch.empty((n, m), dtype=torch.int32, device=dev)
    det_score = torch.empty((n, m), dtype=torch.float32, device=dev)
    det_idx = torch.empty((n, m), dtype=torch.int32, device=dev)
    det_count = torch.empty((n,), dtype=torch.int32, device=dev)
    C.call("dle_ssd_select_fwd", C.ptr(boxes), C.ptr(kept_idx), C.ptr(kept_score), C.ptr(kept_count), C.ptr(det_boxes),
           C.ptr(det_label), C.ptr(det_score), C.ptr(det_idx), C.ptr(det_count), n, b, lm1 + 1, max_num, max_output, C.stream())
    return det_boxes, det_label, det_score, det_idx, det_count


def conv2d_dgrad(dy, w, in_hw, stride=1, pad=0, addend=None, out=None):
    C.require_cuda(dy, w, addend, out)
    n, p, q, ko = dy.shape
    ko2, r, s, c = w.shape
    h, wd = in_hw
    if ko2 != ko or not dy.is_contiguous() or not w.is_contiguous() or (p, q) != _conv_out(h, wd, r, s, stride, pad):
        raise ValueError("conv2d_dgrad: shape mismatch")
    if out is None:
        out = torch.empty((n, h, wd, c), dtype=dy.dtype, device=dy.device)
    if addend is not None and (addend.shape != out.shape or not addend.is_contiguous() or addend.dtype != dy.dtype):
        raise ValueError("conv2d_dgrad: addend must match dx")
    if r == 1 and s == 1 and pad == 0 and stride > 1 and addend is None and c % 8 == 0:
        m = n * p * q
        compact = gemm(dy.view(m, ko), w.view(ko, c), m, c, ko, True, False)
        C.annotate(bytes=float(out.numel() + compact.numel()) * 2, tag="N%dx%dx%dxC%d s%d" % (n, h, wd, c, stride))
        C.call("dle_upsample_zero", C.ptr(compact), C.ptr(out), n, p, q, h, wd, c, stride, C.dt(dy), C.stream())
        return out
    C.annotate(flops=2.0 * n * p * q * ko * r * s * c, tag="dgrad %dx%dx%dx%d k%d %dx%d s%d" % (n, h, wd, c, ko, r, s, stride),
               bytes=float(dy.numel() + w.numel() + out.numel()) * 2)
    if (r == 3 and s == 3 and stride == 2 and pad == 1 and addend is None and h % 2 == 0 and wd % 2 == 0
            and ko % 64 == 0 and c % 8 == 0):
        ws = splitk_workspace(dy.device, 9 * ko * c * 2)
        C.call("dle_conv2d_dgrad_s2", C.ptr(dy), C.ptr(w), C.ptr(out), n, h, wd, c, ko, C.ptr(ws), ws.numel() * 4,
               C.dt(dy), C.stream())
        return out
    C.call("dle_conv2d_dgrad", C.ptr(dy), C.ptr(w), C.ptr(out), C.ptr(addend), n, h, wd, c, ko, r, s, stride, pad,
           C.dt(dy), C.stream())
    return out


def upsample_zero(compact, in_hw, stride):
    C.require_cuda(compact)
    n, p, q, c = compact.shape
    h, wd = in_hw
    out = torch.empty((n, h, wd, c), dtype=compact.dtype, device=compact.device)
    C.annotate(bytes=float(out.numel() + compact.numel()) * 2, tag="N%dx%dx%dxC%d s%d" % (n, h, wd, c, stride))
    C.call("dle_upsample_zero", C.ptr(compact), C.ptr(out), n, p, q, h, wd, c, stride, C.dt(compact), C.stream())
    return out


def _timed_optional(name, fn, args, replayable=True):
    tm = C._timer
    if tm is None:
        return fn(*args)
    s, e = torch.cuda.Event(enable_timing=True), torch.cuda.Event(enable_timing=True)
    s.record()
    rc = fn(*args)
    e.record()
    meta, tm.meta = tm.meta, None
    if rc == 1:
        tm.records.append((name, s, e, meta))
        if replayable:
            tm.last[(name, meta.get("tag") if meta else None)] = (fn, args, torch.cuda.current_stream())
    return rc


def conv1x1_s2_dgrad_compact(dy, w):
    n, p, q, ko = dy.shape
    c = w.shape[-1]
    m = n * p * q
    return gemm(dy.view(m, ko), w.view(ko, c), m, c, ko, True, False).view(n, p, q, c)


def gemm_add_upsampled2(a, b, compact, hw):
    C.require_cuda(a, b, compact)
    m, k = a.shape
    k2, nn = b.shape
    h, wd = hw
    if k2 != k or a.stride(1) != 1 or b.stride(1) != 1 or not compact.is_contiguous() or compact.shape[-1] != nn or \
            a.dtype != b.dtype or compact.dtype != a.dtype:
        raise ValueError("gemm_add_upsampled2: shape / layout mismatch")
    out = torch.empty((m, nn), dtype=a.dtype, device=a.device)
    C.annotate(flops=2.0 * m * nn * k, tag="%dx%dx%d+up2" % (m, nn, k), bytes=float(a.numel() + b.numel() + out.numel() + compact.numel()) * 2)
    rc = _timed_optional("dle_gemm", C.lib().dle_gemm_expand_add_up2,
                         (C.ptr(a), C.ptr(b), C.ptr(out), C.ptr(compact), m, nn, k, a.stride(0), b.stride(0), nn, nn, 0, h, wd, C.dt(a),
                          C.stream()))
    if rc == 0:
        return None
    if rc != 1:
        C.check(rc - 1000 if rc > 1000 else rc, "dle_gemm_expand_add_up2")
    return out


def wgrad1x1(dy2d, x2d, out, accumulate=False):
    C.require_cuda(dy2d, x2d, out)
    m, ko = dy2d.shape
    c = x2d.shape[1]
    if x2d.shape[0] != m or not dy2d.is_contiguous() or not x2d.is_contiguous() or not out.is_contiguous() or \
            out.numel() != ko * c or out.dtype != torch.float32 or dy2d.dtype != x2d.dtype:
        return False
    need = int(C.lib().dle_wgrad1x1_workspace_for(m, ko, c))
    if need == 0:
        return False
    ws = splitk_workspace(dy2d.device, need)
    C.annotate(flops=2.0 * m * ko * c, tag="%dx%dx%d" % (ko, c, m), bytes=float(dy2d.numel() + x2d.numel()) * 2 + out.numel() * 4.0)
    rc = _timed_optional("dle_gemm", C.lib().dle_wgrad1x1_try,
                         (C.ptr(dy2d), C.ptr(x2d), C.ptr(out), m, ko, c, C.dt(dy2d), int(accumulate), C.ptr(ws), ws.numel() * 4, C.stream()),
                         replayable=not accumulate)
    if rc > 1:
        C.check(rc - 1000 if rc > 1000 else -1, "dle_wgrad1x1_try")
    return rc == 1


def conv2d_wgrad(dy, x, rs, stride=1, pad=0, out=None, accumulate=False, splitk=None):
    C.require_cuda(dy, x, out)
    n, p, q, ko = dy.shape
    n2, h, wd, c = x.shape
    r, s = rs
    if n2 != n or not dy.is_contiguous() or not x.is_contiguous() or (p, q) != _conv_out(h, wd, r, s, stride, pad):
        raise ValueError("conv2d_wgrad: shape mismatch")
    if out is None:
        out = torch.empty((ko, r, s, c), dtype=torch.float32, device=x.device)
        accumulate = False
    m_out, n_out, k = ko, r * s * c, n * p * q
    if splitk is None:
        splitk = pick_splitk(m_out, n_out, k, target_blocks=1024)
    need = splitk * m_out * n_out * 4 if splitk > 1 else 0
    if (r, s, stride, pad) == (3, 3, 1, 1):
        need = max(need, int(C.lib().dle_conv3x3_wgrad_workspace()))
    ws = splitk_workspace(x.device, need) if need else None
    C.annotate(flops=2.0 * n * p * q * ko * r * s * c, tag="wgrad %dx%dx%dx%d k%d %dx%d s%d" % (n, h, wd, c, ko, r, s, stride),
               bytes=float(dy.numel() + x.numel()) * 2 + out.numel() * 4.0)
    C.call("dle_conv2d_wgrad", C.ptr(dy), C.ptr(x), C.ptr(out), n, h, wd, c, ko, r, s, stride, pad, C.dt(x), splitk,
           int(accumulate), C.ptr(ws), ws.numel() * 4 if ws is not None else 0, C.stream())
    return out


def nchw_to_nhwc(x, out_dtype, c_padded=None):
    C.require_cuda(x)
    if x.dtype != torch.float32 or x.dim() != 4 or not x.is_contiguous():
        raise ValueError("nchw_to_nhwc expects a contiguous fp32 NCHW tensor")
    n, c, h, w = x.shape
    cp = c_padded or (c + 7) // 8 * 8
    y = torch.empty((n, h, w, cp), dtype=out_dtype, device=x.device)
    C.call("dle_nchw_to_nhwc", C.ptr(x), C.ptr(y), n, c, h * w, cp, C.dt(y), C.stream())
    return y


def u8_nchw_normalize_nhwc(x, mean, std, out_dtype, c_padded=None):
    C.require_cuda(x, mean, std)
    if x.dtype != torch.uint8 or x.dim() != 4 or not x.is_contiguous():
        raise ValueError("u8_nchw_normalize_nhwc expects a contiguous uint8 NCHW tensor")
    n, c, h, w = x.shape
    cp = c_padded or (c + 7) // 8 * 8
    y = torch.empty((n, h, w, cp), dtype=out_dtype, device=x.device)
    C.call("dle_u8_nchw_normalize_nhwc", C.ptr(x), C.ptr(y), C.ptr(mean), C.ptr(std), n, c, h * w, cp, C.dt(y), C.stream())
    return y


def _bn_ws(x2d):
    m, c = x2d.shape
    nbytes = C.lib().dle_bn_workspace_bytes(m, c)
    return splitk_workspace(x2d.device, nbytes)


def bn_fwd(x, gamma, beta, running_mean=None, running_var=None, eps=1e-5, momentum=0.1, residual=None, relu=True,
           out=None, want_mask=False):
    C.require_cuda(x, gamma, beta, running_mean, running_var, residual, out)
    c = x.shape[-1]
    m = x.numel() // c
    x2 = x.reshape(m, c)
    mean = torch.empty(c, dtype=torch.float32, device=x.device)
    rstd = torch.empty(c, dtype=torch.float32, device=x.device)
    ws = _bn_ws(x2)
    C.annotate(bytes=float(x.numel()) * 2, tag="M%dxC%d" % (x.numel() // c, c))
    C.call("dle_bn_fwd_stats", C.ptr(x), m, c, eps, momentum, C.ptr(mean), C.ptr(rstd), C.ptr(running_mean),
           C.ptr(running_var), C.ptr(ws), ws.numel() * 4, C.dt(x), C.stream())
    y = torch.empty_like(x) if out is None else out
    mask = torch.empty(x.numel() // 8, dtype=torch.uint8, device=x.device) if (want_mask and relu) else None
    C.annotate(bytes=float(x.numel()) * (2 * (3 if residual is not None else 2) + (0.125 if mask is not None else 0)),
               tag="M%dxC%d%s" % (x.numel() // c, c, "+res" if residual is not None else ""))
    C.call("dle_bn_fwd_apply", C.ptr(x), C.ptr(residual), C.ptr(y), C.ptr(mask), C.ptr(mean), C.ptr(rstd), C.ptr(gamma),
           C.ptr(beta), m, c, int(relu), C.dt(x), C.stream())
    if want_mask:
        return y, mean, rstd, mask
    return y, mean, rstd


def conv2d_fwd_bnstats(x, w, stride=1, pad=0, running_mean=None, running_var=None, eps=1e-5, momentum=0.1):
    C.require_cuda(x, w, running_mean, running_var)
    n, h, wd, c = x.shape
    ko, r, s, c2 = w.shape
    if c2 != c or not x.is_contiguous() or not w.is_contiguous() or x.dtype != w.dtype:
        raise ValueError("conv2d_fwd_bnstats: x must be NHWC-contiguous and w KRSC-contiguous with matching C/dtype")
    p, q = _conv_out(h, wd, r, s, stride, pad)
    m = n * p * q
    y = torch.empty((n, p, q, ko), dtype=x.dtype, device=x.device)
    groups = max((m + 127) // 128, min(1032, (m + 63) // 64 + 8))
    ws = splitk_workspace(x.device, (groups + 32) * 2 * ko * 4)
    part, fold = ws[:groups * 2 * ko], ws[groups * 2 * ko:(groups + 32) * 2 * ko]
    import ctypes
    g_out = ctypes.c_int(0)
    C.annotate(flops=2.0 * m * ko * r * s * c, tag="fwd+stats %dx%dx%dx%d k%d %dx%d s%d" % (n, h, wd, c, ko, r, s, stride),
               bytes=float(x.numel() + w.numel() + y.numel()) * 2)
    C.call("dle_conv2d_fwd_colstats", C.ptr(x), C.ptr(w), C.ptr(y), n, h, wd, c, ko, r, s, stride, pad, C.dt(x),
           C.ptr(part), part.numel() * 4, ctypes.byref(g_out), C.stream())
    mean = torch.empty(ko, dtype=torch.float32, device=x.device)
    rstd = torch.empty(ko, dtype=torch.float32, device=x.device)
    C.call("dle_bn_stats_from_partials", C.ptr(part), g_out.value, m, ko, float(eps), float(momentum), C.ptr(mean),
           C.ptr(rstd), C.ptr(running_mean), C.ptr(running_var), C.ptr(fold), fold.numel() * 4, C.stream())
    return y, mean, rstd


def conv1x1_bnload_fwd(t, res, w, mean, rstd, gamma, beta, running_mean=None, running_var=None, eps=1e-5, momentum=0.1, res_bn=None):
    C.require_cuda(t, res, w, mean, rstd, gamma, beta, running_mean, running_var, *(res_bn or ()))
    k = t.shape[-1]
    n = w.shape[0]
    m = t.numel() // k
    if not t.is_contiguous() or not w.is_contiguous() or w.numel() != n * k or w.dtype != t.dtype or \
            (res is not None and (res.shape != t.shape or not res.is_contiguous() or res.dtype != t.dtype)):
        raise ValueError("conv1x1_bnload_fwd: dense operands of one 16-bit dtype expected")
    groups = C.lib().dle_conv1x1_bnload_groups(m, n, k)
    if groups == 0:
        return None
    out = torch.empty(t.shape[:-1] + (n,), dtype=t.dtype, device=t.device)
    y = torch.empty_like(t)
    bits = torch.empty(t.numel() // 8, dtype=torch.uint8, device=t.device)
    ws = splitk_workspace(t.device, (groups + 32) * 2 * n * 4)
    part, fold = ws[:groups * 2 * n], ws[groups * 2 * n:(groups + 32) * 2 * n]
    C.annotate(flops=2.0 * m * n * k, tag="bn+conv %dx%dx%d%s" % (m, n, k, "+res" if res is not None else ""),
               bytes=float(t.numel() * (3 if res is not None else 2) + out.numel() + w.numel()) * 2 + bits.numel())
    if res_bn is not None:
        if res is None:
            raise ValueError("conv1x1_bnload_fwd: res_bn without a residual")
        C.annotate(flops=2.0 * m * n * k, tag="bn+conv %dx%dx%d+bnres" % (m, n, k),
                   bytes=float(t.numel() * 3 + out.numel() + w.numel()) * 2 + bits.numel())
        rc = _timed_optional("dle_conv1x1_bnload_fwd", C.lib().dle_conv1x1_bnload_fwd2,
                             (C.ptr(t), C.ptr(res), C.ptr(w), C.ptr(out), C.ptr(y), C.ptr(bits), C.ptr(mean), C.ptr(rstd), C.ptr(gamma),
                              C.ptr(beta), C.ptr(res_bn[0]), C.ptr(res_bn[1]), C.ptr(res_bn[2]), C.ptr(res_bn[3]),
                              C.ptr(part), part.numel() * 4, m, n, k, C.dt(t), C.stream()))
    else:
        rc = _timed_optional("dle_conv1x1_bnload_fwd", C.lib().dle_conv1x1_bnload_fwd,
                             (C.ptr(t), C.ptr(res), C.ptr(w), C.ptr(out), C.ptr(y), C.ptr(bits), C.ptr(mean), C.ptr(rstd), C.ptr(gamma),
                              C.ptr(beta), C.ptr(part), part.numel() * 4, m, n, k, C.dt(t), C.stream()))
    if rc == 0:
        return None
    if rc != 1:
        C.check(rc - 1000 if rc > 1000 else -1, "dle_conv1x1_bnload_fwd")
    mean_o = torch.empty(n, dtype=torch.float32, device=t.device)
    rstd_o = torch.empty(n, dtype=torch.float32, device=t.device)
    C.call("dle_bn_stats_from_partials", C.ptr(part), groups, m, n, float(eps), float(momentum), C.ptr(mean_o), C.ptr(rstd_o),
           C.ptr(running_mean), C.ptr(running_var), C.ptr(fold), fold.numel() * 4, C.stream())
    return out, y, bits, mean_o, rstd_o


def stem_pack_weight(w_master, out_dtype, out=None):
    C.require_cuda(w_master, out)
    ko, ci, r, s = w_master.shape
    phys = w_master.permute(0, 2, 3, 1)
    if (ko, ci, r, s) != (64, 3, 7, 7) or not phys.is_contiguous() or w_master.dtype != torch.float32:
        raise ValueError("stem_pack_weight expects a channels_last fp32 [64, 3, 7, 7] weight")
    if out is None:
        out = torch.empty((64, 7, 8, 4), dtype=out_dtype, device=w_master.device)
    C.call("dle_stem_pack_weight", C.ptr(w_master), C.ptr(out), C.dt(out), C.stream())
    return out


def stem_conv_fwd(x4, w2, want_stats=True):
    C.require_cuda(x4, w2)
    n, h, wd, c = x4.shape
    if c != 4 or not x4.is_contiguous() or tuple(w2.shape) != (64, 7, 8, 4) or w2.dtype != x4.dtype or not w2.is_contiguous():
        raise ValueError("stem_conv_fwd: x4 must be [N, H, W, 4] and w2 the packed [64, 7, 8, 4] weight of the same dtype")
    p, q = (h - 1) // 2 + 1, (wd - 1) // 2 + 1
    y = torch.empty((n, p, q, 64), dtype=x4.dtype, device=x4.device)
    part = None
    if want_stats:
        groups = C.lib().dle_stem_conv7_groups(n, h)
        part = splitk_workspace(x4.device, (groups + 32) * 2 * 64 * 4)[:(groups + 32) * 2 * 64]
    C.annotate(flops=2.0 * n * p * q * 64 * 147, tag="stem fwd%s %dx%dx%d" % ("+stats" if want_stats else "", n, h, wd),
               bytes=float(x4.numel() + y.numel()) * 2)
    C.call("dle_stem_conv7_fwd", C.ptr(x4), C.ptr(w2), C.ptr(y), C.ptr(part), part.numel() * 4 if part is not None else 0, n, h, wd,
           C.dt(x4), C.stream())
    return y, part


def stem_conv_fwd_bnstats(x4, w2, running_mean=None, running_var=None, eps=1e-5, momentum=0.1):
    y, part = stem_conv_fwd(x4, w2, want_stats=True)
    n, p, q, ko = y.shape
    groups = C.lib().dle_stem_conv7_groups(n, x4.shape[1])
    mean = torch.empty(ko, dtype=torch.float32, device=y.device)
    rstd = torch.empty(ko, dtype=torch.float32, device=y.device)
    fold = part[groups * 2 * ko:]
    C.call("dle_bn_stats_from_partials", C.ptr(part), groups, n * p * q, ko, float(eps), float(momentum), C.ptr(mean),
           C.ptr(rstd), C.ptr(running_mean), C.ptr(running_var), C.ptr(fold), fold.numel() * 4, C.stream())
    return y, mean, rstd


def stem_conv_wgrad(dy, x4, out, accumulate=False):
    C.require_cuda(dy, x4, out)
    n, h, wd, c = x4.shape
    if c != 4 or not x4.is_contiguous() or not dy.is_contiguous() or dy.shape[0] != n or dy.shape[3] != 64 or \
            out.numel() != 64 * 147 or out.dtype != torch.float32 or not out.is_contiguous():
        raise ValueError("stem_conv_wgrad: shape mismatch")
    ws = splitk_workspace(x4.device, int(C.lib().dle_stem_conv7_wgrad_workspace(n, h)))
    C.annotate(flops=2.0 * dy.numel() * 147, tag="stem wgrad %dx%dx%d" % (n, h, wd), bytes=float(dy.numel() + x4.numel()) * 2)
    C.call("dle_stem_conv7_wgrad", C.ptr(dy), C.ptr(x4), C.ptr(out), C.ptr(ws), ws.numel() * 4, n, h, wd, C.dt(x4), int(accumulate),
           C.stream())
    return out


def bn_fwd_apply(x, mean, rstd, gamma, beta, residual=None, relu=True, want_mask=False, residual_bn=None):
    C.require_cuda(x, mean, rstd, gamma, beta, residual, *(residual_bn or ()))
    c = x.shape[-1]
    m = x.numel() // c
    y = torch.empty_like(x)
    if residual_bn is not None:
        if residual is None or not relu or not want_mask or residual.shape != x.shape or residual.dtype != x.dtype \
                or not (x.is_contiguous() and residual.is_contiguous()):
            raise ValueError("bn_fwd_apply: residual_bn needs a dense residual of x's shape / dtype, relu and want_mask")
        mask = torch.empty(x.numel() // 8, dtype=torch.uint8, device=x.device)
        C.annotate(bytes=float(x.numel()) * (6 + 0.125), tag="M%dxC%d+bnres" % (m, c))
        C.call("dle_bn_fwd_apply2", C.ptr(x), C.ptr(residual), C.ptr(y), C.ptr(mask), C.ptr(mean), C.ptr(rstd), C.ptr(gamma), C.ptr(beta),
               C.ptr(residual_bn[0]), C.ptr(residual_bn[1]), C.ptr(residual_bn[2]), C.ptr(residual_bn[3]), m, c, C.dt(x), C.stream())
        return y, mask
    mask = torch.empty(x.numel() // 8, dtype=torch.uint8, device=x.device) if (want_mask and relu) else None
    C.annotate(bytes=float(x.numel()) * (2 * (3 if residual is not None else 2) + (0.125 if mask is not None else 0)),
               tag="M%dxC%d%s" % (m, c, "+res" if residual is not None else ""))
    C.call("dle_bn_fwd_apply", C.ptr(x), C.ptr(residual), C.ptr(y), C.ptr(mask), C.ptr(mean), C.ptr(rstd), C.ptr(gamma),
           C.ptr(beta), m, c, int(relu), C.dt(x), C.stream())
    return y, mask


def bn_relu_maxpool_fwd(t, mean, rstd, gamma, beta):
    C.require_cuda(t, mean, rstd, gamma, beta)
    n, h, w, c = t.shape
    if h % 2 or w % 2 or not t.is_contiguous():
        raise ValueError("bn_relu_maxpool_fwd: contiguous NHWC input with even H, W expected")
    y = torch.empty((n, h // 2, w // 2, c), dtype=t.dtype, device=t.device)
    am = torch.empty((n, h // 2, w // 2, c), dtype=torch.uint8, device=t.device)
    mask = torch.empty(t.numel() // 8, dtype=torch.uint8, device=t.device)
    C.annotate(bytes=float(t.numel() + y.numel()) * 2 + am.numel() + mask.numel(), tag="N%dx%dx%dxC%d" % (n, h, w, c))
    C.call("dle_bn_relu_maxpool_fwd", C.ptr(t), C.ptr(y), C.ptr(am), C.ptr(mask), C.ptr(mean), C.ptr(rstd), C.ptr(gamma), C.ptr(beta),
           n, h, w, c, C.dt(t), C.stream())
    return y, am, mask


def bn_bwd(dy, y, x, mean, rstd, gamma, dgamma, dbeta, want_skip_grad=False, dx_out=None, relu_mask=None, reduce_done=False):
    C.require_cuda(dy, y, x, mean, rstd, gamma, dgamma, dbeta, relu_mask)
    c = x.shape[-1]
    m = x.numel() // c
    ws = _bn_ws(x.reshape(m, c))
    if relu_mask is not None:
        y = None
    act_bytes = 0.125 if relu_mask is not None else (2.0 if y is not None else 0.0)
    relu_tag = "+relu" if (y is not None or relu_mask is not None) else ""
    if not reduce_done:
        C.annotate(bytes=float(x.numel()) * (4 + act_bytes), tag="M%dxC%d%s" % (x.numel() // c, c, relu_tag))
        C.call("dle_bn_bwd_reduce", C.ptr(dy), C.ptr(y), C.ptr(relu_mask), C.ptr(x), C.ptr(mean), C.ptr(rstd), C.ptr(dgamma),
               C.ptr(dbeta), m, c, 0, C.ptr(ws), ws.numel() * 4, C.dt(x), C.stream())
    dx = torch.empty_like(x) if dx_out is None else dx_out
    g = torch.empty_like(x) if want_skip_grad else None
    C.annotate(bytes=float(x.numel()) * (6 + act_bytes + 2 * int(want_skip_grad)),
               tag="M%dxC%d%s%s" % (x.numel() // c, c, relu_tag, "+skip" if want_skip_grad else ""))
    C.call("dle_bn_bwd_apply", C.ptr(dy), C.ptr(y), C.ptr(relu_mask), C.ptr(x), C.ptr(dx), C.ptr(g), C.ptr(mean),
           C.ptr(rstd), C.ptr(gamma), C.ptr(dgamma), C.ptr(dbeta), m, c, C.dt(x), C.stream())
    return dx, g


def bn_bwd_reduce2(dy, relu_mask, x1, mean1, rstd1, dgamma1, dbeta1, x2, mean2, rstd2, dgamma2, dbeta2):
    C.require_cuda(dy, relu_mask, x1, mean1, rstd1, dgamma1, dbeta1, x2, mean2, rstd2, dgamma2, dbeta2)
    c = x1.shape[-1]
    m = x1.numel() // c
    if x2.shape != x1.shape or dy.shape != x1.shape or not (dy.is_contiguous() and x1.is_contiguous() and x2.is_contiguous()) \
            or x1.dtype != dy.dtype or x2.dtype != dy.dtype:
        raise ValueError("bn_bwd_reduce2: dy, x1, x2 must be dense tensors of one shape / dtype")
    ws = splitk_workspace(x1.device, 2 * int(C.lib().dle_bn_workspace_bytes(m, c)))
    C.annotate(bytes=float(x1.numel()) * (6 + 0.125), tag="M%dxC%d+relu x2" % (m, c))
    C.call("dle_bn_bwd_reduce2", C.ptr(dy), C.ptr(relu_mask), C.ptr(x1), C.ptr(mean1), C.ptr(rstd1), C.ptr(dgamma1), C.ptr(dbeta1),
           C.ptr(x2), C.ptr(mean2), C.ptr(rstd2), C.ptr(dgamma2), C.ptr(dbeta2), m, c, C.ptr(ws), ws.numel() * 4, C.dt(x1), C.stream())


def gemm_masked_add_bnred(g2, w, m, n, k, addend, bits, t2, bits2, mean2, rstd2, dgamma2, dbeta2):
    C.require_cuda(g2, w, addend, bits, t2, bits2, mean2, rstd2, dgamma2, dbeta2)
    if (g2.dtype not in (torch.float16, torch.bfloat16) or m < 4096 or k not in (64, 128, 256) or n % 128 != 0 or n < 2 * k
            or (k == 256 and os.environ.get("DLE_GEMM_BNRED_K256", "0") != "1")
            or not (g2.is_contiguous() and w.is_contiguous() and addend.is_contiguous() and t2.is_contiguous())
            or t2.numel() != m * n or os.environ.get("DLE_RN50_FUSE_BNRED", "1") == "0"):
        return None
    groups = int(C.lib().dle_gemm_expand_groups(m, n, k))
    if groups <= 0:
        return None
    ws = splitk_workspace(g2.device, groups * 2 * n * 4)
    out = torch.empty((m, n), dtype=g2.dtype, device=g2.device)
    by = float(m) * (k + 3 * n) * g2.element_size() + float(m) * n * 0.25 + float(k) * n * 2
    C.annotate(bytes=by, flops=2.0 * m * n * k, tag="%dx%dx%d+src+aux+bnred" % (m, n, k))
    rc = _timed_optional("dle_gemm", C.lib().dle_gemm_expand_masked_bnred,
                         (C.ptr(g2), C.ptr(w), C.ptr(out), C.ptr(addend), C.ptr(bits), C.ptr(t2), C.ptr(bits2), C.ptr(mean2),
                          C.ptr(rstd2), C.ptr(ws), ws.numel() * 4, m, n, k, g2.stride(0), w.stride(0), out.stride(0), 0, C.dt(g2),
                          C.stream()))
    if rc > 1:
        C.check(rc - 1000 if rc > 1000 else -1, "dle_gemm_expand_masked_bnred")
    if rc != 1:
        return None
    C.call("dle_bn_bwd_finish", C.ptr(ws), groups, n, C.ptr(dgamma2), C.ptr(dbeta2), 0, C.stream())
    return out


def _bn_bwd_conv1x1(dy, x, mean, rstd, gamma, dgamma, dbeta, w, relu_mask, reduce_done, bnred, xin=None, gw=None):
    wg = xin is not None
    more = (xin, gw) if wg else ()
    C.require_cuda(dy, x, mean, rstd, gamma, dgamma, dbeta, w, relu_mask, *more)
    k = x.shape[-1]
    m = x.numel() // k
    n = w.shape[-1]
    if (m < 4096 or k != 256 or n != 64 or w.numel() != k * n or not all(t.is_contiguous() for t in (dy, x, w) + more)
            or x.dtype not in (torch.float16, torch.bfloat16) or dy.dtype != x.dtype or w.dtype != x.dtype
            or (wg and (xin.numel() != m * n or gw.numel() != k * n or gw.dtype != torch.float32 or xin.dtype != x.dtype))
            or os.environ.get("DLE_CONV_BNBWD", "1") == "0"
            or any(t is not None and t.data_ptr() % 16 for t in (dy, x, w, relu_mask) + more)):
        return None
    ws = _bn_ws(x.reshape(m, k))
    act_bytes = 0.125 if relu_mask is not None else 0.0
    relu_tag = "+relu" if relu_mask is not None else ""
    if not reduce_done:
        C.annotate(bytes=float(x.numel()) * (4 + act_bytes), tag="M%dxC%d%s" % (m, k, relu_tag))
        C.call("dle_bn_bwd_reduce", C.ptr(dy), None, C.ptr(relu_mask), C.ptr(x), C.ptr(mean), C.ptr(rstd), C.ptr(dgamma),
               C.ptr(dbeta), m, k, 0, C.ptr(ws), ws.numel() * 4, C.dt(x), C.stream())
    dt = None if wg else torch.empty_like(x)
    dx = torch.empty((m, n), dtype=x.dtype, device=x.device)
    t2 = bits2 = mean2 = rstd2 = part = None
    if bnred is not None and bnred[0].numel() == m * n and bnred[0].is_contiguous() and bnred[1] is not None \
            and os.environ.get("DLE_RN50_FUSE_BNRED", "1") != "0" and os.environ.get("DLE_RN50_FUSE_BNRED2", "1") != "0":
        t2, bits2, mean2, rstd2 = bnred[:4]
    groups = int(C.lib().dle_conv1x1_bnbwd_groups(m)) if wg or t2 is not None else 0
    bnred_tag = "+bnred" if t2 is not None else ""
    if wg:
        name = "dle_conv1x1_bnbwd_dgrad_wgrad"
        wg_bytes = int(C.lib().dle_conv1x1_bnbwd_wgrad_workspace(m, int(t2 is not None)))
        part_bytes = (groups * 2 * n * 4 + 15) // 16 * 16 if t2 is not None else 0
        buf = splitk_workspace(x.device, part_bytes + wg_bytes)
        part = buf[:part_bytes // 4] if t2 is not None else None
        wpart = buf[part_bytes // 4:]
        C.annotate(bytes=float(x.numel()) * (4 + act_bytes) + (dx.numel() + xin.numel()) * 2.0
                   + dx.numel() * (2.125 if t2 is not None else 0.0),
                   flops=4.0 * m * n * k, tag="bn_bwd+dgrad+wgrad %dx%dx%d%s%s" % (m, n, k, relu_tag, bnred_tag))
        args = (C.ptr(dy), C.ptr(x), C.ptr(relu_mask), C.ptr(w), C.ptr(dx), C.ptr(mean), C.ptr(rstd), C.ptr(gamma), C.ptr(dgamma),
                C.ptr(dbeta), C.ptr(t2), C.ptr(bits2), C.ptr(mean2), C.ptr(rstd2), C.ptr(part), part_bytes, C.ptr(xin), C.ptr(gw),
                C.ptr(wpart), wpart.numel() * 4, m, n, k, C.dt(x), C.stream())
    else:
        name = "dle_conv1x1_bnbwd_dgrad"
        if t2 is not None:
            part = splitk_workspace(x.device, groups * 2 * n * 4)
        C.annotate(bytes=float(x.numel()) * (6 + act_bytes) + dx.numel() * (2.0 + (2.125 if t2 is not None else 0.0)),
                   flops=2.0 * m * n * k, tag="bn_bwd+dgrad %dx%dx%d%s%s" % (m, n, k, relu_tag, bnred_tag))
        args = (C.ptr(dy), C.ptr(x), C.ptr(relu_mask), C.ptr(w), C.ptr(dt), C.ptr(dx), C.ptr(mean), C.ptr(rstd), C.ptr(gamma),
                C.ptr(dgamma), C.ptr(dbeta), C.ptr(t2), C.ptr(bits2), C.ptr(mean2), C.ptr(rstd2), C.ptr(part),
                part.numel() * 4 if part is not None else 0, m, n, k, C.dt(x), C.stream())
    rc = _timed_optional(name, getattr(C.lib(), name), args)
    if rc > 1:
        C.check(rc - 1000 if rc > 1000 else -1, name)
    if rc != 1:
        dt, _ = bn_bwd(dy, None, x, mean, rstd, gamma, dgamma, dbeta, relu_mask=relu_mask, reduce_done=True, dx_out=dt)
        gemm(dt.view(m, k), w, m, n, k, True, False, out=dx)
        if wg and not wgrad1x1(dt.view(m, k), xin.view(m, n), gw.view(k, n)):
            gemm(dt.view(m, k), xin.view(m, n), k, n, m, False, False, out=gw.view(k, n),
                 splitk=pick_splitk(k, n, m, target_blocks=1024))
        return (None if wg else dt), dx, False
    if t2 is not None:
        C.call("dle_bn_bwd_finish", C.ptr(part), groups, n, C.ptr(bnred[4]), C.ptr(bnred[5]), 0, C.stream())
    return dt, dx, t2 is not None


def bn_bwd_conv1x1_dgrad(dy, x, mean, rstd, gamma, dgamma, dbeta, w, relu_mask=None, reduce_done=False, bnred=None):
    return _bn_bwd_conv1x1(dy, x, mean, rstd, gamma, dgamma, dbeta, w, relu_mask, reduce_done, bnred)


def bn_bwd_conv1x1_dgrad_wgrad(dy, x, mean, rstd, gamma, dgamma, dbeta, w, xin, gw, relu_mask=None, reduce_done=False, bnred=None):
    out = _bn_bwd_conv1x1(dy, x, mean, rstd, gamma, dgamma, dbeta, w, relu_mask, reduce_done, bnred, xin, gw)
    return out and out[1:]


def maxpool_fwd(x, ksize=3, stride=2, pad=1):
    C.require_cuda(x)
    n, h, w, c = x.shape
    p, q = (h + 2 * pad - ksize) // stride + 1, (w + 2 * pad - ksize) // stride + 1
    y = torch.empty((n, p, q, c), dtype=x.dtype, device=x.device)
    am = torch.empty((n, p, q, c), dtype=torch.uint8, device=x.device)
    C.annotate(bytes=float(x.numel() + y.numel()) * 2 + am.numel())
    C.call("dle_maxpool_fwd", C.ptr(x), C.ptr(y), C.ptr(am), n, h, w, c, ksize, stride, pad, C.dt(x), C.stream())
    return y, am


def maxpool_bwd(dy, argmax, in_hw, ksize=3, stride=2, pad=1):
    C.require_cuda(dy, argmax)
    n, p, q, c = dy.shape
    h, w = in_hw
    dx = torch.empty((n, h, w, c), dtype=dy.dtype, device=dy.device)
    C.annotate(bytes=float(dx.numel() + dy.numel()) * 2 + argmax.numel())
    C.call("dle_maxpool_bwd", C.ptr(dy), C.ptr(argmax), C.ptr(dx), n, h, w, c, ksize, stride, pad, C.dt(dy), C.stream())
    return dx


def pool_bn_bwd(dy, argmax, x, mean, rstd, gamma, dgamma, dbeta, relu_mask):
    C.require_cuda(dy, argmax, x, mean, rstd, gamma, dgamma, dbeta, relu_mask)
    n, h, w, c = x.shape
    if relu_mask is None or dy.shape != (n, h // 2, w // 2, c) or not (dy.is_contiguous() and x.is_contiguous()) or dy.dtype != x.dtype:
        return None
    nbytes = int(C.lib().dle_pool_bn_bwd_workspace_bytes(n, h, w, c))
    if nbytes == 0:
        return None
    ws = splitk_workspace(x.device, nbytes)
    dz = torch.empty_like(x)
    C.annotate(bytes=2.0 * (dy.numel() * 3 + x.numel() * 2.125) + x.numel() * 2.0, tag="N%dx%dx%dxC%d" % (n, h, w, c))
    C.call("dle_pool_bn_bwd", C.ptr(dy), C.ptr(argmax), C.ptr(relu_mask), C.ptr(x), C.ptr(dz), C.ptr(mean), C.ptr(rstd), C.ptr(gamma),
           C.ptr(dgamma), C.ptr(dbeta), n, h, w, c, C.ptr(ws), ws.numel() * 4, C.dt(x), C.stream())
    return dz


def avgpool_fwd(x):
    C.require_cuda(x)
    n, h, w, c = x.shape
    y = torch.empty((n, c), dtype=x.dtype, device=x.device)
    C.call("dle_avgpool_fwd", C.ptr(x), C.ptr(y), n, h * w, c, C.dt(x), C.stream())
    return y


def avgpool_bwd(dy, hw):
    C.require_cuda(dy)
    n, c = dy.shape
    h, w = hw
    dx = torch.empty((n, h, w, c), dtype=dy.dtype, device=dy.device)
    C.call("dle_avgpool_bwd", C.ptr(dy), C.ptr(dx), n, h * w, c, C.dt(dy), C.stream())
    return dx


def softmax_xent(logits, target, smoothing=0.0, ignore_index=-100, grad_scale=None, grad_dtype=None, ld_out=None):
    C.require_cuda(logits, target, grad_scale)
    if logits.dtype != torch.float32 or logits.dim() != 2 or logits.stride(1) != 1 or target.dtype != torch.int64:
        raise ValueError("softmax_xent expects fp32 [rows, classes] logits and int64 targets")
    rows, classes = logits.shape
    loss = torch.empty(1, dtype=torch.float32, device=logits.device)
    scratch = torch.empty(1, dtype=torch.int32, device=logits.device)
    dl = None
    ldo = ld_out or classes
    if grad_dtype is not None:
        dl = torch.empty((rows, ldo), dtype=grad_dtype, device=logits.device)
    C.call("dle_softmax_xent", C.ptr(logits), C.ptr(target), C.ptr(loss), C.ptr(dl), C.ptr(grad_scale), C.ptr(scratch),
           rows, classes, logits.stride(0), ldo, float(smoothing), int(ignore_index),
           C.dt(grad_dtype) if grad_dtype is not None else 0, C.stream())
    return loss, dl


def gemm_batched(a, b, c, m, n, k, lda, ldb, ldc, a_kc, b_kc, batch, batch_inner, sa, sb, sc, alpha=1.0):
    C.require_cuda(a, b, c)
# ... 1266 lines not shown
```

### include/dle_mi355x.h

```cpp
#ifndef DLE_MI355X_H
#define DLE_MI355X_H
#include <stdint.h>

#ifdef __cplusplus
extern "C" {
#endif

typedef struct ihipStream_t* hipStream_t;

enum { DLE_F32 = 0, DLE_F16 = 1, DLE_BF16 = 2 };
enum { DLE_ACT_NONE = 0, DLE_ACT_RELU = 1, DLE_ACT_GELU = 2, DLE_ACT_RELU_BWD = 3, DLE_ACT_ADD = 4,
       DLE_ACT_GELU_BWD = 5, DLE_ACT_TANH = 6, DLE_ACT_TANH_BWD = 7,
       DLE_ACT_ADD_MASKED = 8,
       DLE_ACT_MUL = 9,
       DLE_ACT_GELU_DAUX = 10   };

const char* dle_last_error(void);
int dle_abi_version(void);
int dle_device_check(int device, char* arch_name, int arch_name_len);

int dle_dot_interact_out_width(int rows, int cols);
int dle_dot_interact_fwd(const void* x, void* out, int batch, int rows, int cols, int dtype,
                         int force_generic, hipStream_t stream);
int dle_dot_interact_bwd(const void* x, const void* upstream, void* grad, void* mlp_grad,
// ... 61 lines not shown
                     int64_t sc_i, hipStream_t stream);

int dle_conv2d_fwd(const void* x, const void* w, void* y, const float* bias, int N, int H, int W, int C,
                   int Ko, int R, int S, int stride, int pad, int dtype, int out_dtype, int act,
                   hipStream_t stream);
int dle_conv2d_dgrad(const void* dy, const void* w, void* dx, const void* addend, int N, int H, int W, int C,
                     int Ko, int R, int S, int stride, int pad, int dtype, hipStream_t stream);
int dle_conv2d_fwd_affine(const void* x, const void* w, void* y, const float* scale, const float* shift,
                          const void* residual, int N, int H, int W, int C, int Ko, int R, int S, int stride, int pad,
                          int dtype, int relu, hipStream_t stream);
int64_t dle_conv3x3_affine_launch_count(void);
int dle_conv2d_grouped_fwd_affine(const void* x, const void* w, void* y, const float* scale, const float* shift,
                                  int N, int H, int W, int C, int Ko, int groups, int stride,
                                  int dtype, int relu, hipStream_t stream);
int dle_se_gate(const void* t, const float* w1, const float* b1, const float* w2, const float* b2, float* gate,
                int N, int HW, int C, int S, int dtype, hipStream_t stream);
int dle_se_apply(const void* t, const float* gate, const void* residual, void* y,
                 int64_t N, int HW, int C, int dtype, int relu, hipStream_t stream);
#define DLE_DWCONV_TILE_ROWS 8
#define DLE_DWCONV_TILE_COLS 16
#define DLE_DWCONV_CHUNK 64
int dle_dwconv2d_act_fwd(const void* x, const void* w, void* y, const float* scale, const float* shift, float* pool,
                         int64_t pool_bytes, int N, int H, int W, int C, int ksize, int stride, int in_act, int out_act,
                         int dtype, hipStream_t stream);
int dle_dwconv2d_pool_bands(int H, int W, int C, int ksize, int stride);
#define DLE_SE_GATE_ACT_MAX_C_PLUS_S 16384
int dle_se_gate_act(const float* pool, int G, float inv_hw, const float* w1, const float* b1, const float* w2,
                    const float* b2, float* gate, int N, int C, int S, int act, hipStream_t stream);
int dle_silu_avgpool_fwd(const void* x, void* y, int N, int HW, int C, int dtype, hipStream_t stream);
#define DLE_SSD_MAX_MAPS 8
#define DLE_SSD_MAX_KEEP 256
#define DLE_SSD_MAX_BOXES 16384
int dle_ssd_decode_fwd(const void* const* heads, const int* geom, int nmaps, const float* dboxes_xywh, float* boxes, float* probs,
                       int N, int B, int L, float scale_xy, float scale_wh, int dtype, hipStream_t stream);
int dle_ssd_nms_fwd(const float* boxes, const float* probs, int* kept_idx, float* kept_score, int* kept_count, int N, int B, int L,
                    float threshold, float criteria, int max_num, hipStream_t stream);
int dle_ssd_select_fwd(const float* boxes, const int* kept_idx, const float* kept_score, const int* kept_count, float* det_boxes,
                       int* det_label, float* det_score, int* det_idx, int* det_count, int N, int B, int L, int max_num,
                       int max_output, hipStream_t stream);
int dle_conv2d_wgrad(const void* dy, const void* x, float* dw, int N, int H, int W, int C, int Ko, int R, int S,
                     int stride, int pad, int dtype, int splitk, int accumulate, void* workspace,
                     int64_t workspace_bytes, hipStream_t stream);
int64_t dle_wgrad1x1_workspace(void);
int dle_wgrad1x1_mode(int mode);
int64_t dle_wgrad1x1_workspace_for(int M, int Ko, int C);
int dle_wgrad1x1_try(const void* dy, const void* x, float* dw, int M, int Ko, int C, int dtype, int accumulate, void* workspace,
                     int64_t workspace_bytes, hipStream_t stream);
int64_t dle_conv3x3_wgrad_workspace(void);
int dle_conv3x3_wgrad_mode(int mode);

int dle_colsum(const void* x, float* out, int64_t M, int N, int64_t ld, int dtype, int accumulate,
               void* workspace, int64_t workspace_bytes, hipStream_t stream);
int64_t dle_colsum_batched_workspace_bytes(int n, int64_t M, int N);
int dle_colsum_batched(const int64_t* table_dev, int n, int64_t M, int N, int64_t ld, int dtype, void* workspace,
                       int64_t workspace_bytes, hipStream_t stream);

int64_t dle_mt_table_len(int n_tensors, int n_lists);
int64_t dle_mt_table_fill(int64_t* table_host, int n_tensors, int n_lists, const int64_t* sizes,
                          const void* const* ptrs, int chunk);
int dle_mt_l2norm(const int64_t* table_dev, int n_tensors, int64_t total_chunks, int chunk, int dtype,
                  float* partial_scratch, float* ret, float* ret_per_tensor, int per_tensor,
                  int* noop_flag, hipStream_t stream);
int dle_mt_lamb_stage1(const int64_t* table_dev, int n_tensors, int64_t total_chunks, int chunk,
                       int grad_dtype, const int* noop_flag, float beta1, float beta2, float beta3,
                       const int* step_dev, int bias_correction, float eps, int mode,
                       float weight_decay, const float* global_grad_norm, const float* max_grad_norm,
                       const float* inv_scale, hipStream_t stream);
int dle_mt_lamb_stage1_norms(const int64_t* table_dev, int n_tensors, int64_t total_chunks, int chunk, int grad_dtype,
                             int* noop_flag, float beta1, float beta2, float beta3, const int* step_dev, int bias_correction,
                             float eps, int mode, float weight_decay, const float* global_grad_norm, const float* max_grad_norm,
                             const float* inv_scale, float* partial, float* param_norm, float* update_norm, hipStream_t stream);
int dle_mt_lamb_stage2(const int64_t* table_dev, int n_tensors, int64_t total_chunks, int chunk,
                       int grad_dtype, int copy_dtype, const int* noop_flag,
                       const float* param_norm, const float* update_norm, const float* lr_dev,
                       float weight_decay, int use_nvlamb, hipStream_t stream);
int dle_mt_sgd(const int64_t* table_dev, int n_tensors, int64_t total_chunks, int chunk, int grad_dtype,
               int has_momentum, const float* skip_flag_dev, const float* lr_dev, float lr_host,
               float momentum, float dampening, float weight_decay, int nesterov, int first_step,
               const float* inv_scale_dev, int copy_dtype, hipStream_t stream);

int dle_cast_rows(const void* in, void* out, int64_t rows, int cols, int cols_out, int64_t ld_in,
                  int64_t ld_out, int in_dtype, int out_dtype, hipStream_t stream);
int dle_transpose_cast(const void* x, void* y, int rows, int cols, int64_t ld_x, int64_t ld_y, int in_dtype, int out_dtype,
                       hipStream_t stream);
int dle_a2a_blocks(void* blocks, void* x, int rows, int world, const int* widths, int elem_size, int pack, hipStream_t stream);
int dle_bce_logits(const void* logits, const float* target, float* loss_out, void* dlogits,
                   const float* grad_scale_dev, int64_t n, int64_t ld_logits, int dtype, hipStream_t stream);
int dle_gemm_colsum(const void* A, const void* B, void* C, const void* src, float* colsum_out, int M, int N, int K, int64_t lda,
                    int64_t ldb, int64_t ldc, int dtype, int act, int accumulate_colsum, void* workspace,
                    int64_t workspace_bytes, hipStream_t stream);
int64_t dle_head_bce_workspace_bytes(int64_t M, int K);
int dle_head_bce_fwd_bwd(const void* h, const void* w16, const float* bias, const float* target,
                         const float* grad_scale_dev, float* loss_out, void* logits_out, void* dh, float* gw, float* gb,
                         float* gprev_bias, void* ws, int64_t ws_bytes, int64_t M, int K, int64_t ldh, int64_t ldd,
                         int dtype, hipStream_t stream);
int dle_amp_update_scale(float* scale, int* growth_tracker, float* found_inf, float* inv_scale,
                         float growth_factor, float backoff_factor, int growth_interval,
                         int clear_found_inf, hipStream_t stream);
int dle_check_nonfinite(const void* x, float* found_inf, int64_t n, int dtype, hipStream_t stream);
int dle_axpby_f32(const float* x, const float* y, float* out, float a, float b, int64_t n, hipStream_t stream);
int dle_act_bwd(const void* g, const void* src, void* out, int64_t n, int act, int dtype, hipStream_t stream);
int dle_relu_bwd(const void* g, const void* y, void* out, int64_t rows, int cols, int64_t ld_g, int64_t ld_y,
                 int64_t ld_out, int dtype, hipStream_t stream);

int dle_nchw_to_nhwc(const float* x, void* y, int64_t N, int C, int64_t HW, int C_padded, int out_dtype,
                     hipStream_t stream);
int64_t dle_bn_workspace_bytes(int64_t M, int C);
int dle_bn_fwd_stats(const void* x, int64_t M, int C, float eps, float momentum, float* mean, float* rstd,
                     float* running_mean, float* running_var, void* workspace, int64_t workspace_bytes,
                     int dtype, hipStream_t stream);
int dle_conv2d_fwd_colstats(const void* x, const void* w, void* y, int N, int H, int W, int C, int Ko, int R, int S,
                            int stride, int pad, int dtype, float* col_partial, int64_t col_partial_bytes,
                            int* groups, hipStream_t stream);
int dle_bn_stats_from_partials(const float* partial, int groups, int64_t M, int C, float eps, float momentum,
                               float* mean, float* rstd, float* running_mean, float* running_var, void* workspace,
                               int64_t workspace_bytes, hipStream_t stream);
int dle_bn_fwd_apply(const void* x, const void* residual, void* y, void* relu_mask, const float* mean,
                     const float* rstd, const float* gamma, const float* beta, int64_t M, int C, int relu,
                     int dtype, hipStream_t stream);
int dle_bn_fwd_apply2(const void* x, const void* xr, void* y, void* relu_mask, const float* mean, const float* rstd,
                      const float* gamma, const float* beta, const float* mean_r, const float* rstd_r, const float* gamma_r,
                      const float* beta_r, int64_t M, int C, int dtype, hipStream_t stream);
int dle_bn_bwd_reduce(const void* dy, const void* y, const void* relu_mask, const void* x, const float* mean,
                      const float* rstd, float* dgamma, float* dbeta, int64_t M, int C, int accumulate,
                      void* workspace, int64_t workspace_bytes, int dtype, hipStream_t stream);
int dle_bn_bwd_reduce2(const void* dy, const void* relu_mask, const void* x1, const float* mean1, const float* rstd1, float* dgamma1,
                       float* dbeta1, const void* x2, const float* mean2, const float* rstd2, float* dgamma2, float* dbeta2,
                       int64_t M, int C, void* workspace, int64_t workspace_bytes, int dtype, hipStream_t stream);
int dle_bn_bwd_apply(const void* dy, const void* y, const void* relu_mask, const void* x, void* dx, void* g_out,
                     const float* mean, const float* rstd, const float* gamma, const float* dgamma,
                     const float* dbeta, int64_t M, int C, int dtype, hipStream_t stream);
int dle_conv1x1_bnload_groups(int M, int N, int K);
int dle_conv1x1_bnload_fwd(const void* t, const void* res, const void* w, void* out, void* y, void* bits, const float* mean,
                           const float* rstd, const float* gamma, const float* beta, float* stats, int64_t stats_bytes, int M,
                           int N, int K, int dtype, hipStream_t stream);
int dle_conv1x1_bnload_fwd2(const void* t, const void* res, const void* w, void* out, void* y, void* bits, const float* mean,
                            const float* rstd, const float* gamma, const float* beta, const float* mean_r, const float* rstd_r,
                            const float* gamma_r, const float* beta_r, float* stats, int64_t stats_bytes, int M, int N, int K,
                            int dtype, hipStream_t stream);
int dle_conv1x1_bnbwd_dgrad(const void* dy, const void* t, const void* relu_mask, const void* w, void* dt, void* dx,
                            const float* mean, const float* rstd, const float* gamma, const float* dgamma, const float* dbeta,
                            const void* t2, const void* bits2, const float* mean2, const float* rstd2, float* partial,
                            int64_t partial_bytes, int M, int N, int K, int dtype, hipStream_t stream);
int dle_conv1x1_bnbwd_groups(int M);
int dle_conv1x1_bnbwd_dgrad_wgrad(const void* dy, const void* t, const void* relu_mask, const void* w, void* dx,
                                  const float* mean, const float* rstd, const float* gamma, const float* dgamma,
                                  const float* dbeta, const void* t2, const void* bits2, const float* mean2, const float* rstd2,
                                  float* partial, int64_t partial_bytes, const void* x, float* gw, void* workspace,
                                  int64_t workspace_bytes, int M, int N, int K, int dtype, hipStream_t stream);
int64_t dle_conv1x1_bnbwd_wgrad_workspace(int M, int bnred);
int dle_gemm_expand_masked_bnred(const void* A, const void* B, void* C, const void* src, const void* bits, const void* t2,
                                 const void* bits2, const float* mean2, const float* rstd2, float* partial, int64_t partial_bytes,
                                 int M, int N, int K, int64_t lda, int64_t ldb, int64_t ldc, int b_kc, int dtype, hipStream_t stream);
int dle_bn_bwd_finish(const float* partial, int groups, int C, float* dgamma, float* dbeta, int accumulate, hipStream_t stream);
int dle_stem_conv7_groups(int N, int H);
int dle_stem_conv7_fwd(const void* x4, const void* w2, void* y, float* stats, int64_t stats_bytes, int N, int H, int W,
                       int dtype, hipStream_t stream);
int64_t dle_stem_conv7_wgrad_workspace(int N, int H);
int dle_stem_conv7_wgrad(const void* dy, const void* x4, float* dw, void* workspace, int64_t workspace_bytes, int N, int H,
                         int W, int dtype, int accumulate, hipStream_t stream);
int dle_stem_pack_weight(const float* w_krsc, void* out, int dtype, hipStream_t stream);
int dle_maxpool_fwd(const void* x, void* y, void* argmax, int N, int H, int W, int C, int ksize, int stride,
                    int pad, int dtype, hipStream_t stream);
int dle_bn_relu_maxpool_fwd(const void* x, void* y, void* argmax, void* relu_mask, const float* mean, const float* rstd,
                            const float* gamma, const float* beta, int N, int H, int W, int C, int dtype, hipStream_t stream);
int dle_maxpool_bwd(const void* dy, const void* argmax, void* dx, int N, int H, int W, int C, int ksize,
                    int stride, int pad, int dtype, hipStream_t stream);
int64_t dle_pool_bn_bwd_workspace_bytes(int N, int H, int W, int C);
int dle_pool_bn_bwd(const void* dy, const void* argmax, const void* relu_mask, const void* x, void* dz, const float* mean,
                    const float* rstd, const float* gamma, float* dgamma, float* dbeta, int N, int H, int W, int C, void* workspace,
                    int64_t workspace_bytes, int dtype, hipStream_t stream);
int dle_avgpool_fwd(const void* x, void* y, int64_t N, int HW, int C, int dtype, hipStream_t stream);
int dle_avgpool_bwd(const void* dy, void* dx, int64_t N, int HW, int C, int dtype, hipStream_t stream);
int dle_gemm_expand_add_up2(const void* A, const void* B, void* C, const void* compact, int M, int N, int K, int64_t lda,
                            int64_t ldb, int64_t ldc, int64_t ld_compact, int b_kc, int H, int W, int dtype, hipStream_t stream);
int dle_upsample_zero(const void* x, void* y, int64_t N, int P, int Q, int H, int W, int C, int stride, int dtype,
                      hipStream_t stream);
int dle_softmax_xent(const float* logits, const int64_t* target, float* loss_out, void* dlogits,
                     const float* grad_scale_dev, int* scratch, int64_t rows, int classes, int64_t ld,
                     int64_t ld_out, float smoothing, int64_t ignore_index, int dlogits_dtype,
                     hipStream_t stream);

int dle_layernorm_fwd(const void* x, const void* residual, void* z_out, void* y, const float* gamma,
                      const float* beta, float* mean, float* rstd, int64_t rows, int H, float eps, int dtype,
                      hipStream_t stream);
int64_t dle_layernorm_workspace_bytes(int H);
int dle_layernorm_bwd(const void* dy, const void* z, const float* mean, const float* rstd, const float* gamma,
                      void* dz, float* dgamma, float* dbeta, int64_t rows, int H, int accumulate, void* workspace,
                      int64_t workspace_bytes, int dtype, hipStream_t stream);
int dle_embed_sum(const float* word, const float* pos, const float* type, const int64_t* ids,
                  const int64_t* token_type, void* z, int64_t tokens, int S, int H, int dtype, hipStream_t stream);
int dle_embed_sum_packed(const float* word, const float* pos, const float* type, const int64_t* ids,
                         const int64_t* token_type, const int32_t* position_ids, void* z, int64_t tokens, int H, int dtype,
                         hipStream_t stream);
int dle_embed_scatter_add(const void* dz, const int64_t* ids, float* grad_word, int64_t tokens, int H, int dtype,
                          hipStream_t stream);
int dle_rows_select_sum(const void* x, const int64_t* sel, float* out, int64_t rows, int H, int K, int accumulate,
                        void* workspace, int64_t workspace_bytes, int dtype, hipStream_t stream);
int dle_rows_gather(const void* src, const int64_t* idx, void* dst, int64_t n, int H, int dtype, hipStream_t stream);
int dle_rows_scatter(const void* src, const int64_t* idx, void* dst, int64_t n, int H, int accumulate, int dtype,
                     hipStream_t stream);
int dle_softmax_fwd(void* scores, const float* mask_add, int64_t rows, int L, int rows_per_batch, float scale,
                    int dtype, hipStream_t stream);
int dle_softmax_bwd(const void* probs, void* dprobs, int64_t rows, int L, float scale, int dtype,
                    hipStream_t stream);

int dle_dropout_add_layernorm_bwd(const void* dy, const void* z, const float* mean, const float* rstd, const float* gamma,
                                  const void* keep_mask, float p, void* dz, void* dx, float* dgamma, float* dbeta,
                                  float* dbias, int64_t rows, int H, int accumulate, void* workspace,
                                  int64_t workspace_bytes, int dtype, hipStream_t stream);
int dle_dropout_fwd(const void* x, void* y, void* mask, int64_t n, float p, uint64_t seed, uint64_t offset,
                    const uint64_t* offset_base,
                    int dtype, hipStream_t stream);
int dle_dropout_bwd(const void* dy, const void* mask, void* dx, int64_t n, float p, int dtype, hipStream_t stream);
int dle_dropout_add_layernorm_fwd(const void* x, const void* residual, void* z_out, void* y, void* mask,
                                  const float* gamma, const float* beta, float* mean, float* rstd, int64_t rows,
                                  int H, float eps, float p, uint64_t seed, uint64_t offset,
                                  const uint64_t* offset_base, int dtype,
                                  hipStream_t stream);
int dle_softmax_dropout_fwd(void* scores, void* dropped, void* mask, const float* mask_add, int64_t rows, int L,
                            int rows_per_batch, float scale, float p, uint64_t seed, uint64_t offset,
                            const uint64_t* offset_base, int dtype,
                            hipStream_t stream);
int dle_softmax_dropout_bwd(const void* probs, void* dprobs, const void* mask, int64_t rows, int L, float scale,
                            float p, int dtype, hipStream_t stream);

int dle_u8_nchw_normalize_nhwc(const void* x, void* y, const float* mean, const float* std, int64_t N, int C, int64_t HW,
                               int C_padded, int out_dtype, hipStream_t stream);

int dle_conv2d_dgrad_s2(const void* dy, const void* w, void* dx, int N, int H, int W, int C, int Ko, void* workspace,
                        int64_t workspace_bytes, int dtype, hipStream_t stream);

int dle_attention_supported(int S, int head_dim);
int dle_attention_stats_floats(int S);
int dle_attention_fwd(const void* qkv, const float* mask_add, void* ctx, float* stats, void* keep_mask, int B, int S,
                      int heads, int head_dim, float scale, float p, uint64_t seed, uint64_t offset,
                      const uint64_t* offset_base, int dtype,
                      hipStream_t stream);
int dle_attention_bwd(const void* qkv, const void* dctx, const float* mask_add, const float* stats, void* dqkv,
                      float* colsum_partial, int B, int S, int heads, int head_dim, float scale, float p, uint64_t seed,
                      uint64_t offset, const uint64_t* offset_base, int dtype, hipStream_t stream);
int dle_attention_bwd_keep(const void* qkv, const void* dctx, const float* mask_add, const float* stats, const void* keep_mask,
                           void* dqkv, float* colsum_partial, int B, int S, int heads, int head_dim, float scale, float p,
                           uint64_t seed, uint64_t offset, const uint64_t* offset_base, int dtype, hipStream_t stream);

int dle_attention_varlen_supported(int max_seqlen, int head_dim);
int dle_attention_fwd_varlen(const void* qkv, const int32_t* cu_seqlens, void* ctx, int B, int max_seqlen,
                             int64_t total_tokens, int heads, int head_dim, float scale, int dtype, hipStream_t stream);
uint64_t dle_attention_varlen_launch_count(void);

int dle_mt_adam(const int64_t* table_dev, int n_tensors, int64_t total_chunks, int chunk, const float* skip_flag_dev,
                const float* lr_dev, float lr_host, float beta1, float beta2, float eps, float weight_decay,
                const int* step_dev, const float* inv_scale_dev, const float* grad_norm_dev, float max_grad_norm,
                hipStream_t stream);

int dle_mt_adam_copy(const int64_t* table_dev, int n_tensors, int64_t total_chunks, int chunk, int copy_dtype,
                     const float* skip_flag_dev, const float* lr_dev, float lr_host, float beta1, float beta2, float eps,
                     const int* step_dev, const float* inv_scale_dev, const float* tensor_mul_dev, hipStream_t stream);

int dle_mt_ema(const int64_t* table_dev, int n_tensors, int64_t total_chunks, int chunk, const float* coef_dev, float mu_host,
               float one_minus_mu_host, hipStream_t stream);

int dle_wg_taps(const void* x, void* col, int B, int T, int C, int ntaps, int dilation, int left, int64_t ld_x, int dtype,
                hipStream_t stream);
int dle_wg_taps_bwd(const void* dcol, const void* addend, void* dx, int B, int T, int C, int ntaps, int dilation, int left,
                    int64_t ld_add, int64_t ld_dx, int dtype, hipStream_t stream);
int dle_wg_gate_fwd(const void* s, void* acts, int64_t M, int nc, int64_t ld_s, int dtype, hipStream_t stream);
int dle_wg_gate_bwd(const void* dacts, const void* s, void* ds, int64_t M, int nc, int64_t ld_s, int64_t ld_ds, int dtype,
                    hipStream_t stream);
int dle_wg_invconv_fwd(const float* x, const float* W, float* y, void* a0_16, int64_t M, int c, int dtype,
                       hipStream_t stream);
int dle_wg_invconv_bwd_partials(int64_t M);
int dle_wg_invconv_bwd(const float* dy, const float* da0, const float* x, const float* W, const float* WinvT, float* dx,
                       float* dW, const float* scale_dev, float logdet_coef, float* workspace, int64_t M, int c,
                       hipStream_t stream);
int dle_wg_logdet_inv(const float* W, float* logdet, float* WinvT, float* sign, int c, hipStream_t stream);
int dle_wg_coupling_partials(int64_t M);
int dle_wg_coupling_fwd(const float* y, const float* o, float* z, float* logs_partial, int64_t M, int c, hipStream_t stream);
int dle_wg_coupling_bwd(const float* dz, const float* y, const float* o, float* dy, void* d_o16, const float* scale_dev,
                        float logs_coef, int64_t M, int c, int dtype, hipStream_t stream);
int dle_wg_loss(const float* z, const float* logs_partial, int n_logs, const float* logdets, int n_flows, float sigma,
                int64_t M, float* loss_out, float* workspace, hipStream_t stream);
int dle_wg_dz_init(const float* z, float* dz, const float* scale_dev, float coef, int64_t M, hipStream_t stream);
int dle_wg_weight_norm_fwd(const float* v, const float* g, void* w16, int Co, int Ci, int Kt, int Cip, int dtype,
                           hipStream_t stream);
int dle_wg_weight_norm_bwd(const float* dw, const float* v, const float* g, float* dv, float* dg, int Co, int Ci, int Kt,
                           int Cip, hipStream_t stream);
int dle_wg_upsample_weight(const float* w, const float* bias, void* b16, float* bias_rep, int Cm, int ksize, int stride,
                           int dtype, hipStream_t stream);
int dle_wg_upsample_weight_bwd(const float* db, float* dw, int Cm, int ksize, int stride, hipStream_t stream);
int dle_wg_weight_norm_fwd_batched(const int64_t* table_dev, int n_entries, int64_t total_rows, int dtype, hipStream_t stream);
int dle_wg_weight_norm_bwd_batched(const int64_t* table_dev, int n_entries, int64_t total_rows, hipStream_t stream);
int dle_wg_logdet_inv_batched(const float* base, const int64_t* table_dev, float* logdets, float* WinvT, float* signs,
                              int n_flows, hipStream_t stream);
int dle_wg_flow_inv(const float* state, const float* o, const float* WinvT, const float* noise, float* out, void* a0_16,
                    int64_t M, int c, int early, int z_col, float sigma, int next_c, int dtype, hipStream_t stream);
int dle_wg_flow_inv_first(const float* noise, float* out, void* a0_16, int64_t M, int c, float sigma, int dtype,
                          hipStream_t stream);

int dle_t2_tanh_fwd(const void* x, void* y, int64_t n, int dtype, hipStream_t stream);
int dle_t2_lstm_fwd(void* gates, int64_t ld_g, const float* c_prev, float* c_out, void* d0, int64_t ld0, void* d1, int64_t ld1,
                    void* d2, int64_t ld2, const void* keep, int64_t keep_index, float inv_keep, const float* live,
                    const void* h_prev, int64_t ld_hp, void* out_dst, int64_t ld_out, int B, int H, int dtype, hipStream_t stream);
int dle_t2_lstm_gemm_fwd(const void* x, int64_t ldx, const void* w, int64_t ldw, const float* bias, const void* addend,
                         const float* c_prev, float* c_out, void* gates, int64_t ld_g, void* d0, int64_t ld0, void* d1, int64_t ld1,
                         void* d2, int64_t ld2, const void* keep, int64_t keep_index, float inv_keep, int B, int H, int K, int dtype,
                         hipStream_t stream);
int dle_t2_lstm_bwd(const float* dh, int64_t ld_dh, const float* dh1, int64_t ld_dh1, const float* dh2, int64_t ld_dh2,
                    const float* dc_next, const void* act, int64_t ld_act, const float* c_prev,
                    void* dgates, int64_t ld_dg, float* dc_prev, const void* keep, int64_t keep_index, float inv_keep,
                    const float* live, float* dh_prev, int B, int H, int dtype, hipStream_t stream);
int dle_t2_attention_fwd(const float* q, const void* pl, const float* v, const void* memory, const int64_t* lengths,
                         const void* awc_prev, void* tanh_out, float* aw_out, void* awc_next, void* d0, int64_t ld0, void* d1,
                         int64_t ld1, void* d2, int64_t ld2, const void* wloc, int KL, int KK, int B, int Ti, int A, int E, int dtype,
                         hipStream_t stream);
int dle_t2_attention_bwd(const float* d_ctx0, int64_t ld_c0, const float* d_ctx1, int64_t ld_c1, const float* d_ctx2, int64_t ld_c2,
                         const float* d_aw0, const float* d_aw1, const float* aw, const void* tanh_out, const float* v,
                         const void* memory, float* d_memory, void* d_pl, float* dq, void* dq16, void* dctx16, float* dv_acc,
                         float* d_pm_acc, const void* wlocT, int KL, int KK, float* d_prev, float* d_cum, int B, int Ti, int A, int E,
                         int dtype, hipStream_t stream);
int dle_t2_sum_steps(const void* x, float* out, int n_steps, int64_t R, int dtype, hipStream_t stream);
int dle_t2_location_bwd(const void* dcol, float* d_prev, float* d_cum, int B, int Ti, int KL, int dtype, hipStream_t stream);
int dle_t2_mel_loss(const float* out_all, int64_t ld_out, const void* post, const float* target, const float* scale_dev,
                    void* d_out, int64_t ld_dout, void* d_post, float* loss, float* workspace, int64_t R, int n_mel, int dtype,
                    hipStream_t stream);
int dle_t2_mask_rows(void* x, int64_t ld, int cols, const int64_t* lengths, int64_t B, int To, float value, int dtype,
                     hipStream_t stream);

// ... 128 lines not shown
```

Measured before the change: 13430 samples/s.

## Fuse previous block's BN-backward reduction into upsampled-add expand GEMM and enable K256

```diff
diff --git a/deeplearningexamples_amd/_cabi.py b/deeplearningexamples_amd/_cabi.py
--- a/deeplearningexamples_amd/_cabi.py
+++ b/deeplearningexamples_amd/_cabi.py
@@ -56,6 +56,7 @@
                                               c_void_p]),
     "dle_conv1x1_bnbwd_wgrad_workspace": (c_i64, [c_int, c_int]),
     "dle_gemm_expand_masked_bnred": (c_int, [c_void_p] * 10 + [c_i64, c_int, c_int, c_int, c_i64, c_i64, c_i64, c_int, c_int, c_void_p]),
+    "dle_gemm_expand_masked_bnred2": (c_int, [c_void_p] * 10 + [c_i64, c_int, c_int, c_int, c_i64, c_i64, c_i64, c_int, c_int, c_void_p]),
     "dle_bn_bwd_finish": (c_int, [c_void_p, c_int, c_int, c_void_p, c_void_p, c_int, c_void_p]),
     "dle_gemm_colsum": (c_int, [c_void_p, c_void_p, c_void_p, c_void_p, c_void_p, c_int, c_int, c_int, c_i64, c_i64, c_i64, c_int,
                                 c_int, c_int, c_void_p, c_i64, c_void_p]),
@@ -90,6 +91,8 @@
     "dle_nchw_to_nhwc": (c_int, [c_void_p, c_void_p, c_i64, c_int, c_i64, c_int, c_int, c_void_p]),
     "dle_gemm_expand_add_up2": (c_int, [c_void_p, c_void_p, c_void_p, c_void_p, c_int, c_int, c_int, c_i64, c_i64, c_i64, c_i64, c_int,
                                         c_int, c_int, c_int, c_void_p]),
+    "dle_gemm_expand_add_up2_bnred": (c_int, [c_void_p] * 9 + [c_i64, c_int, c_int, c_int, c_i64, c_i64, c_i64, c_i64, c_int, c_int, c_int,
+                                              c_int, c_void_p]),
     "dle_conv1x1_bnload_groups": (c_int, [c_int, c_int, c_int]),
     "dle_conv1x1_bnload_fwd": (c_int, [c_void_p] * 11 + [c_i64, c_int, c_int, c_int, c_int, c_void_p]),
     "dle_bn_relu_maxpool_fwd": (c_int, [c_void_p] * 8 + [c_int, c_int, c_int, c_int, c_int, c_void_p]),
diff --git a/deeplearningexamples_amd/convnets/engine.py b/deeplearningexamples_amd/convnets/engine.py
--- a/deeplearningexamples_amd/convnets/engine.py
+++ b/deeplearningexamples_amd/convnets/engine.py
@@ -117,6 +117,7 @@
         self.fuse_up2 = os.environ.get("DLE_RN50_FUSE_UP2", "1") != "0"
         self.fuse_bn = os.environ.get("DLE_RN50_FUSE_BN", "1") != "0"
         self.fuse_bnred = os.environ.get("DLE_RN50_FUSE_BNRED", "1") != "0"
+        self.fuse_bnred_up2 = self.fuse_bnred and self.fuse_up2 and os.environ.get("DLE_RN50_FUSE_BNRED_UP2", "1") != "0"
         self.fuse_dsbn = os.environ.get("DLE_RN50_FUSE_DSBN", "1") != "0"
         self.fuse_dsred = os.environ.get("DLE_RN50_FUSE_DSRED", "1") != "0"
         self.fuse_pool_bwd = os.environ.get("DLE_RN50_FUSE_POOLBWD", "1") != "0"
@@ -343,7 +344,7 @@
                 cur.wait_stream(bs)
             if ud is not None:
                 self._done(ud)
-            prev3 = self.blocks[bi - 1][2] if (self.fuse_bnred and ud is None and bi > 0) else None
+            prev3 = self.blocks[bi - 1][2] if (bi > 0 and (self.fuse_bnred if ud is None else self.fuse_bnred_up2)) else None
             g = u1.backward(g2, dx_addend=gskip, bnred=prev3)
             self._done(u1)
         if self.fuse_pool_bwd:
diff --git a/deeplearningexamples_amd/convnets/resnet.py b/deeplearningexamples_amd/convnets/resnet.py
--- a/deeplearningexamples_amd/convnets/resnet.py
+++ b/deeplearningexamples_amd/convnets/resnet.py
@@ -186,7 +186,15 @@
                                  mask_src=dx_addend[0].view(m, c), aux=dx_addend[1])).view(n, h, w, c)
                 else:
                     if up2:
-                        dx = F.gemm_add_upsampled2(g2, self.w16.view(self.cout, c), dx_addend[1], dx_addend[2])
+                        dx = None
+                        if bnred is not None and bnred.saved is not None and bnred.relu and bnred.saved[1].numel() == m * c:
+                            _, pt, pmask, pmean, prstd = bnred.saved
+                            dx = F.gemm_add_upsampled2_bnred(g2, self.w16.view(self.cout, c), dx_addend[1], dx_addend[2],
+                                                             pt.view(m, c), pmask, pmean, prstd, bnred.ggamma, bnred.gbeta)
+                            if dx is not None:
+                                bnred.reduce_done = True
+                        if dx is None:
+                            dx = F.gemm_add_upsampled2(g2, self.w16.view(self.cout, c), dx_addend[1], dx_addend[2])
                         if dx is not None:
                             return dx.view(n, h, w, c)
                         dx_addend = F.upsample_zero(dx_addend[1], dx_addend[2], 2)
diff --git a/deeplearningexamples_amd/csrc/gemm_expand.hip b/deeplearningexamples_amd/csrc/gemm_expand.hip
--- a/deeplearningexamples_amd/csrc/gemm_expand.hip
+++ b/deeplearningexamples_amd/csrc/gemm_expand.hip
@@ -1,4 +1,5 @@
 #include "gemm_tiles.h"
+#include <type_traits>
 
 #define EX_TN 128
 #define EX_PAD 8
@@ -46,19 +47,21 @@
   ushort8_t tv[BRED ? 4 : 1];
   uint4_t mb;
   uint4_t mb2;
-  long long o0;
+  typedef typename std::conditional<BRED && KS == 8, unsigned, long long>::type Off;
+  Off o0;
   bool live;
   bool has;
+  static constexpr bool LATE_T = BRED && KS == 8;
   __device__ __forceinline__ void load_a(const ExpandArgs& p, int m, int kg) {
-    const long long mr = m < p.M ? m : p.M - 1;
-    const unsigned short* arow = p.A + mr * p.lda + kg * 8;
+    const Off mr = m < p.M ? m : p.M - 1;
+    const unsigned short* arow = p.A + (Off)(mr * (Off)p.lda + kg * 8);
 #pragma unroll
     for (int ks = 0; ks < KS; ++ks) fa[ks] = *(const ushort8_t*)(arow + ks * 32);
   }
   __device__ __forceinline__ void load_src(const ExpandArgs& p, int m, int n0, int kg) {
     live = m < p.M;
-    const long long mr = live ? m : p.M - 1;
-    o0 = mr * p.ldc + n0 + kg * 8;
+    const Off mr = live ? m : p.M - 1;
+    o0 = mr * (Off)p.ldc + n0 + kg * 8;
     if (ACT == 3) {
       const int mi = (int)mr;
       const int n = fd_div(mi, p.dHW), rem = mi - n * p.up_HW;
@@ -72,12 +75,17 @@
 #pragma unroll
       for (int j = 0; j < 4; ++j) sv[j] = *(const ushort8_t*)(p.src + o0 + 32 * j);
     }
-    if (ACT == 2) mb = *(const uint4_t*)(p.bits + ((mr * p.ldc + n0) >> 3));
-    if (BRED) {
+    if (ACT == 2) mb = *(const uint4_t*)(p.bits + ((Off)(mr * (Off)p.ldc + n0) >> 3));
+    if (BRED && !LATE_T) {
 #pragma unroll
       for (int j = 0; j < 4; ++j) tv[j] = *(const ushort8_t*)(p.t2 + o0 + 32 * j);
-      mb2 = *(const uint4_t*)(p.bits2 + ((mr * p.ldc + n0) >> 3));
-    }
+      mb2 = *(const uint4_t*)(p.bits2 + ((Off)(mr * (Off)p.ldc + n0) >> 3));
+    }
+  }
+  __device__ __forceinline__ void load_t(const ExpandArgs& p, int kg) {
+#pragma unroll
+    for (int j = 0; j < 4; ++j) tv[j] = *(const ushort8_t*)(p.t2 + o0 + 32 * j);
+    mb2 = *(const uint4_t*)(p.bits2 + ((Off)(o0 - kg * 8) >> 3));
   }
 };
 
@@ -106,10 +114,40 @@
   }
 }
 
+template <int X>
+__device__ __forceinline__ float ex_dpp_xor(float v) {
+  constexpr int ctrl = X == 1 ? 0xB1 : X == 2 ? 0x4E : 0x128;
+  static_assert(X == 1 || X == 2 || X == 8, "DPP forms of lane ^ 1, 2, 8 only");
+  return __int_as_float(__builtin_amdgcn_update_dpp(0, __float_as_int(v), ctrl, 0xf, 0xf, false));
+}
+
+__device__ __forceinline__ void ex_reduce_scatter16_half(const float* v, int fr, float& acc) {
+  float w8[8], w4[4], w2[2];
+  const bool h8 = fr & 8, h4 = fr & 4, h2 = fr & 2, h1 = fr & 1;
+#pragma unroll
+  for (int q = 0; q < 8; ++q) {
+    const float keep = h8 ? v[8 + q] : v[q], send = h8 ? v[q] : v[8 + q];
+    w8[q] = keep + ex_dpp_xor<8>(send);
+  }
+#pragma unroll
+  for (int q = 0; q < 4; ++q) {
+    const float keep = h4 ? w8[4 + q] : w8[q], send = h4 ? w8[q] : w8[4 + q];
+    w4[q] = keep + __shfl_xor(send, 4, 64);
+  }
+#pragma unroll
+  for (int q = 0; q < 2; ++q) {
+    const float keep = h2 ? w4[2 + q] : w4[q], send = h2 ? w4[q] : w4[2 + q];
+    w2[q] = keep + ex_dpp_xor<2>(send);
+  }
+  const float keep = h1 ? w2[1] : w2[0], send = h1 ? w2[0] : w2[1];
+  acc += keep + ex_dpp_xor<1>(send);
+}
+
 template <int DT, int KS, int ACT, bool STATS, int NW, bool BRED = false>
-__global__ __launch_bounds__(NW * 64) __attribute__((amdgpu_waves_per_eu((STATS || BRED) ? 3 : 4)))
+__global__ __launch_bounds__(NW * 64) __attribute__((amdgpu_waves_per_eu((STATS || (BRED && KS != 8)) ? 3 : 4)))
 void gemm_expand_kernel(ExpandArgs p) {
   constexpr int K = KS * 32, LDW = K + EX_PAD, TM = NW * 16;
+  constexpr bool LATE_T = ExStream<KS, ACT, BRED>::LATE_T;
   extern __shared__ __attribute__((aligned(16))) unsigned char smem_raw[];
   unsigned short* wl = (unsigned short*)smem_raw;
   const int lane = threadIdx.x & 63, wave = threadIdx.x >> 6;
@@ -155,6 +193,7 @@
     for (int b = 0; b < 8; ++b) acc[b] = (float4_t){0.f, 0.f, 0.f, 0.f};
 #pragma unroll
     for (int ks = 0; ks < KS; ++ks) {
+      if (LATE_T && ks == KS - 2) cur.load_t(p, kg);
 #pragma unroll
       for (int b = 0; b < 8; ++b) {
         const ushort8_t fw = *(const ushort8_t*)(wrow + b * 16 * LDW + ks * 32);
@@ -162,11 +201,16 @@
       }
       __builtin_amdgcn_sched_barrier(0);
     }
-    cur.load_a(p, m_next, kg);
+    if (!LATE_T) cur.load_a(p, m_next, kg);
     ushort8_t outv[4];
-    float tg[BRED ? 32 : 1], tx[BRED ? 32 : 1];
+    float tg[(BRED && !LATE_T) ? 32 : 1], tx[(BRED && !LATE_T) ? 32 : 1];
     const bool live_cur = cur.live;
     const bool has_cur = ACT == 3 ? cur.has : true;
+    unsigned mbp = 0, mb2p = 0;
+    if (LATE_T && ACT == 2) {
+#pragma unroll
+      for (int j = 0; j < 4; ++j) mbp |= ((cur.mb[j] >> (8 * kg)) & 0xffu) << (8 * j);
+    }
 #pragma unroll
     for (int j = 0; j < 4; ++j) {
       float v[8];
@@ -175,7 +219,7 @@
       if (ACT) {
         float y[8];
         unpack8<DT>(cur.sv[j], y);
-        const unsigned int bits8 = ACT == 2 ? (cur.mb[j] >> (8 * kg)) & 0xffu : 0xffu;
+        const unsigned int bits8 = ACT == 2 ? (LATE_T ? (mbp >> (8 * j)) & 0xffu : (cur.mb[j] >> (8 * kg)) & 0xffu) : 0xffu;
 #pragma unroll
         for (int r = 0; r < 8; ++r) {
           if (ACT == 2) { if ((bits8 >> r) & 1u) v[r] += y[r]; }
@@ -195,7 +239,7 @@
           s2[8 * j + r] += zz * zz;
         }
       }
-      if (BRED) {
+      if (BRED && !LATE_T) {
         float z[8], tf[8];
         unpack8<DT>(ov, z);
         unpack8<DT>(cur.tv[j], tf);
@@ -211,7 +255,47 @@
         }
       }
     }
-    if (BRED) {
+    if (LATE_T) {
+#pragma unroll
+      for (int j = 0; j < 4; ++j) mb2p |= ((cur.mb2[j] >> (8 * kg)) & 0xffu) << (8 * j);
+#pragma unroll
+      for (int h = 0; h < 2; ++h) {
+        float tv16[16];
+#pragma unroll
+        for (int x = 0; x < 2; ++x) {
+#pragma unroll
+          for (int jj = 0; jj < 2; ++jj) {
+            const int j = 2 * h + jj;
+            float z[8], tf[8];
+            if (x) {
+              uint4_t o = __builtin_bit_cast(uint4_t, outv[j]);
+              asm volatile("" : "+v"(o[0]), "+v"(o[1]), "+v"(o[2]), "+v"(o[3]));
+              outv[j] = __builtin_bit_cast(ushort8_t, o);
+            }
+            unpack8<DT>(outv[j], z);
+            const unsigned b2 = (mb2p >> (8 * j)) & 0xffu;
+#pragma unroll
+            for (int r = 0; r < 8; ++r) z[r] = (live_cur && ((b2 >> r) & 1u)) ? z[r] : 0.f;
+            if (x) {
+              unpack8<DT>(cur.tv[j], tf);
+              const float4_t m0 = *(const float4_t*)(mu2 + 32 * j + 8 * kg), m1 = *(const float4_t*)(mu2 + 32 * j + 8 * kg + 4);
+              const float4_t r0 = *(const float4_t*)(mu2 + EX_TN + 32 * j + 8 * kg), r1 = *(const float4_t*)(mu2 + EX_TN + 32 * j + 8 * kg + 4);
+#pragma unroll
+              for (int r = 0; r < 8; ++r) {
+                const float mu = r < 4 ? m0[r & 3] : m1[r & 3], rs = r < 4 ? r0[r & 3] : r1[r & 3];
+                z[r] = z[r] * (tf[r] - mu) * rs;
+              }
+            }
+#pragma unroll
+            for (int r = 0; r < 8; ++r) tv16[8 * jj + r] = z[r];
+          }
+          ex_reduce_scatter16_half(tv16, fr, x ? b2s[h] : b1[h]);
+          __builtin_amdgcn_sched_barrier(0);
+        }
+      }
+      cur.load_a(p, m_next, kg);
+    }
+    if (BRED && !LATE_T) {
       ex_reduce_scatter16(tg, fr, b1);
       ex_reduce_scatter16(tx, fr, b2s);
     }
@@ -222,8 +306,9 @@
       const bool odd = fr & 1;
       const int m_cur = tm * TM + mrow;
       const bool live_other = (odd ? m_cur - 1 : m_cur + 1) < p.M;
-      const long long o_own = (long long)m_cur * p.ldc + n0 + kg * 8;
-      const long long o_other = odd ? o_own - p.ldc : o_own + p.ldc;
+      typedef typename ExStream<KS, ACT, BRED>::Off Off;
+      const Off o_own = (Off)m_cur * (Off)p.ldc + n0 + kg * 8;
+      const Off o_other = odd ? o_own - (Off)p.ldc : o_own + (Off)p.ldc;
 #pragma unroll
       for (int h = 0; h < 2; ++h) {
         const uint4_t mine0 = __builtin_bit_cast(uint4_t, outv[2 * h]), mine1 = __builtin_bit_cast(uint4_t, outv[2 * h + 1]);
@@ -232,8 +317,8 @@
 #pragma unroll
         for (int q = 0; q < 4; ++q) got[q] = (unsigned)__shfl_xor((int)give[q], 1, 64);
         const uint4_t first = odd ? got : mine0, second = odd ? mine1 : got;
-        const long long o_first = (odd ? o_other : o_own) + 64 * h + (odd ? 32 : 0);
-        const long long o_second = (odd ? o_own : o_other) + 64 * h + (odd ? 32 : 0);
+        const Off o_first = (odd ? o_other : o_own) + 64 * h + (odd ? 32 : 0);
+        const Off o_second = (odd ? o_own : o_other) + 64 * h + (odd ? 32 : 0);
         const bool live_first = odd ? live_other : live_cur, live_second = odd ? live_cur : live_other;
         if (live_first) *(uint4_t*)(p.C + o_first) = first;
         if (live_second) *(uint4_t*)(p.C + o_second) = second;
@@ -245,7 +330,7 @@
     float* red = (float*)smem_raw;
 #pragma unroll
     for (int b = 0; b < 2; ++b) {
-      const int i = 2 * fr + b, col = 32 * (i >> 3) + 8 * kg + (i & 7);
+      const int i = LATE_T ? 16 * b + fr : 2 * fr + b, col = 32 * (i >> 3) + 8 * kg + (i & 7);
       red[(wave * 2 + 0) * EX_TN + col] = b1[b];
       red[(wave * 2 + 1) * EX_TN + col] = b2s[b];
     }
@@ -342,13 +427,17 @@
   return 1;
 }
 
-extern "C" int dle_gemm_expand_masked_bnred(const void* A, const void* B, void* C, const void* src, const void* bits, const void* t2,
-                                            const void* bits2, const float* mean2, const float* rstd2, float* partial,
-                                            int64_t partial_bytes, int M, int N, int K, int64_t lda, int64_t ldb, int64_t ldc,
-                                            int b_kc, int dtype, hipStream_t stream) {
+static int ex_bnred_k256() { return dle_env_int("DLE_GEMM_BNRED_K256", 1); }
+static bool ex_offsets_fit32(int M, int64_t lda, int64_t ldc) {
+  return ((int64_t)M + 1) * ldc < (1ll << 31) && ((int64_t)M + 1) * lda < (1ll << 31);
+}
+
+static int ex_masked_bnred(const void* A, const void* B, void* C, const void* src, const void* bits, const void* t2, const void* bits2,
+                           const float* mean2, const float* rstd2, float* partial, int64_t partial_bytes, int M, int N, int K,
+                           int64_t lda, int64_t ldb, int64_t ldc, int b_kc, int dtype, int k256, hipStream_t stream) {
   if (!dle_gemm_expand_enabled()) return 0;
-  const int k256 = dle_env_int("DLE_GEMM_BNRED_K256", 0);
   if (M < 4096 || (K != 64 && K != 128 && !(K == 256 && k256)) || (N % EX_TN) != 0 || N < 2 * K) return 0;
+  if (K == 256 && !ex_offsets_fit32(M, lda, ldc)) return 0;
   if (dtype != DLE_F16 && dtype != DLE_BF16) return 0;
   if (!A || !B || !C || !src || !bits || !t2 || !bits2 || !mean2 || !rstd2 || !partial) return 0;
   if (((((uintptr_t)A) | ((uintptr_t)B) | ((uintptr_t)C) | ((uintptr_t)src) | ((uintptr_t)t2) | ((uintptr_t)bits) | ((uintptr_t)bits2)) & 15) != 0 ||
@@ -377,6 +466,21 @@
   hipError_t e = hipGetLastError();
   if (e != hipSuccess) { dle_set_error("gemm_expand_masked_bnred launch failed: %s", hipGetErrorString(e)); return (int)e + 1000; }
   return 1;
+}
+
+extern "C" int dle_gemm_expand_masked_bnred(const void* A, const void* B, void* C, const void* src, const void* bits, const void* t2,
+                                            const void* bits2, const float* mean2, const float* rstd2, float* partial,
+                                            int64_t partial_bytes, int M, int N, int K, int64_t lda, int64_t ldb, int64_t ldc,
+                                            int b_kc, int dtype, hipStream_t stream) {
+  return ex_masked_bnred(A, B, C, src, bits, t2, bits2, mean2, rstd2, partial, partial_bytes, M, N, K, lda, ldb, ldc, b_kc, dtype,
+                         dle_env_int("DLE_GEMM_BNRED_K256", 0), stream);
+}
+extern "C" int dle_gemm_expand_masked_bnred2(const void* A, const void* B, void* C, const void* src, const void* bits, const void* t2,
+                                             const void* bits2, const float* mean2, const float* rstd2, float* partial,
+                                             int64_t partial_bytes, int M, int N, int K, int64_t lda, int64_t ldb, int64_t ldc,
+                                             int b_kc, int dtype, hipStream_t stream) {
+  return ex_masked_bnred(A, B, C, src, bits, t2, bits2, mean2, rstd2, partial, partial_bytes, M, N, K, lda, ldb, ldc, b_kc, dtype,
+                         ex_bnred_k256(), stream);
 }
 
 extern "C" int dle_gemm_expand_add_up2(const void* A, const void* B, void* C, const void* compact, int M, int N, int K, int64_t lda,
@@ -411,3 +515,40 @@
   if (e != hipSuccess) { dle_set_error("gemm_expand_add_up2 launch failed: %s", hipGetErrorString(e)); return (int)e + 1000; }
   return 1;
 }
+
+extern "C" int dle_gemm_expand_add_up2_bnred(const void* A, const void* B, void* C, const void* compact, const void* t2,
+                                             const void* bits2, const float* mean2, const float* rstd2, float* partial,
+                                             int64_t partial_bytes, int M, int N, int K, int64_t lda, int64_t ldb, int64_t ldc,
+                                             int64_t ld_compact, int b_kc, int H, int W, int dtype, hipStream_t stream) {
+  if (!dle_gemm_expand_enabled()) return 0;
+  if (M < 4096 || !(K == 128 || (K == 256 && ex_bnred_k256())) || (N % EX_TN) != 0 || N < 2 * K) return 0;
+  if (dtype != DLE_F16 && dtype != DLE_BF16) return 0;
+  if ((H & 1) || (W & 1) || H <= 0 || W <= 0 || (M % (H * W)) != 0) return 0;
+  if (!A || !B || !C || !compact || !t2 || !bits2 || !mean2 || !rstd2 || !partial) return 0;
+  if (((((uintptr_t)A) | ((uintptr_t)B) | ((uintptr_t)C) | ((uintptr_t)compact) | ((uintptr_t)t2) | ((uintptr_t)bits2)) & 15) != 0 ||
+      (lda & 7) || (ldb & 7) || (ldc % EX_TN) != 0 || (ld_compact & 7))
+    return 0;
+  if (K == 256 && !ex_offsets_fit32(M, lda, ldc)) return 0;
+  ExpandArgs p = {(const unsigned short*)A, (const unsigned short*)B, (unsigned short*)C, (const unsigned short*)compact, nullptr,
+                  partial, M, N, K, (long long)lda, (long long)ldb, (long long)ldc, b_kc, 0, 0, 0};
+  p.dHW = make_fastdiv(H * W); p.dW = make_fastdiv(W);
+  p.up_HW = H * W; p.up_W = W; p.up_P = H / 2; p.up_Q = W / 2; p.ld_src = ld_compact;
+  p.t2 = (const unsigned short*)t2; p.bits2 = (const unsigned char*)bits2; p.mean2 = mean2; p.rstd2 = rstd2;
+  const int tmr = ex_rows_per_tile(K);
+  p.row_tiles = (M + tmr - 1) / tmr;
+  p.col_tiles = N / EX_TN;
+  p.groups = dle_gemm_expand_groups(M, N, K);
+  if (partial_bytes < (long long)p.groups * 2 * N * 4) return 0;
+  size_t lds_bytes = (size_t)EX_TN * (K + EX_PAD) * 2 + 2 * EX_TN * 4;
+  const dim3 grid((unsigned)(p.groups * p.col_tiles)), block(tmr * 4);
+  if (dtype == DLE_F16) {
+    if (K == 128) DLE_LAUNCH_LDS((gemm_expand_kernel<DLE_F16, 4, 3, false, 4, true>), grid, block, lds_bytes, stream, p);
+    else DLE_LAUNCH_LDS((gemm_expand_kernel<DLE_F16, 8, 3, false, 8, true>), grid, block, lds_bytes, stream, p);
+  } else {
+    if (K == 128) DLE_LAUNCH_LDS((gemm_expand_kernel<DLE_BF16, 4, 3, false, 4, true>), grid, block, lds_bytes, stream, p);
+    else DLE_LAUNCH_LDS((gemm_expand_kernel<DLE_BF16, 8, 3, false, 8, true>), grid, block, lds_bytes, stream, p);
+  }
+  hipError_t e = hipGetLastError();
+  if (e != hipSuccess) { dle_set_error("gemm_expand_add_up2_bnred launch failed: %s", hipGetErrorString(e)); return (int)e + 1000; }
+  return 1;
+}
diff --git a/deeplearningexamples_amd/functional.py b/deeplearningexamples_amd/functional.py
--- a/deeplearningexamples_amd/functional.py
+++ b/deeplearningexamples_amd/functional.py
@@ -912,6 +912,36 @@
     return out
 
 
+def gemm_add_upsampled2_bnred(a, b, compact, hw, t2, bits2, mean2, rstd2, dgamma2, dbeta2):
+    C.require_cuda(a, b, compact, t2, bits2, mean2, rstd2, dgamma2, dbeta2)
+    m, k = a.shape
+    k2, nn = b.shape
+    h, wd = hw
+    if k2 != k or a.stride(1) != 1 or b.stride(1) != 1 or not compact.is_contiguous() or compact.shape[-1] != nn or \
+            a.dtype != b.dtype or compact.dtype != a.dtype:
+        raise ValueError("gemm_add_upsampled2_bnred: shape / layout mismatch")
+    if (a.dtype not in (torch.float16, torch.bfloat16) or k not in (128, 256) or t2.dtype != a.dtype or not t2.is_contiguous()
+            or t2.numel() != m * nn or (k == 256 and os.environ.get("DLE_GEMM_BNRED_K256", "1") == "0")
+            or os.environ.get("DLE_RN50_FUSE_BNRED", "1") == "0"):
+        return None
+    groups = int(C.lib().dle_gemm_expand_groups(m, nn, k))
+    if groups <= 0:
+        return None
+    ws = splitk_workspace(a.device, groups * 2 * nn * 4)
+    out = torch.empty((m, nn), dtype=a.dtype, device=a.device)
+    by = float(a.numel() + b.numel() + 2 * out.numel() + compact.numel()) * 2 + out.numel() * 0.125
+    C.annotate(flops=2.0 * m * nn * k, tag="%dx%dx%d+up2+bnred" % (m, nn, k), bytes=by)
+    rc = _timed_optional("dle_gemm", C.lib().dle_gemm_expand_add_up2_bnred,
+                         (C.ptr(a), C.ptr(b), C.ptr(out), C.ptr(compact), C.ptr(t2), C.ptr(bits2), C.ptr(mean2), C.ptr(rstd2),
+                          C.ptr(ws), ws.numel() * 4, m, nn, k, a.stride(0), b.stride(0), nn, nn, 0, h, wd, C.dt(a), C.stream()))
+    if rc > 1:
+        C.check(rc - 1000 if rc > 1000 else -1, "dle_gemm_expand_add_up2_bnred")
+    if rc != 1:
+        return None
+    C.call("dle_bn_bwd_finish", C.ptr(ws), groups, nn, C.ptr(dgamma2), C.ptr(dbeta2), 0, C.stream())
+    return out
+
+
 def wgrad1x1(dy2d, x2d, out, accumulate=False):
     C.require_cuda(dy2d, x2d, out)
     m, ko = dy2d.shape
@@ -1203,7 +1233,7 @@
 def gemm_masked_add_bnred(g2, w, m, n, k, addend, bits, t2, bits2, mean2, rstd2, dgamma2, dbeta2):
     C.require_cuda(g2, w, addend, bits, t2, bits2, mean2, rstd2, dgamma2, dbeta2)
     if (g2.dtype not in (torch.float16, torch.bfloat16) or m < 4096 or k not in (64, 128, 256) or n % 128 != 0 or n < 2 * k
-            or (k == 256 and os.environ.get("DLE_GEMM_BNRED_K256", "0") != "1")
+            or (k == 256 and os.environ.get("DLE_GEMM_BNRED_K256", "1") == "0")
             or not (g2.is_contiguous() and w.is_contiguous() and addend.is_contiguous() and t2.is_contiguous())
             or t2.numel() != m * n or os.environ.get("DLE_RN50_FUSE_BNRED", "1") == "0"):
         return None
@@ -1214,12 +1244,12 @@
     out = torch.empty((m, n), dtype=g2.dtype, device=g2.device)
     by = float(m) * (k + 3 * n) * g2.element_size() + float(m) * n * 0.25 + float(k) * n * 2
     C.annotate(bytes=by, flops=2.0 * m * n * k, tag="%dx%dx%d+src+aux+bnred" % (m, n, k))
-    rc = _timed_optional("dle_gemm", C.lib().dle_gemm_expand_masked_bnred,
+    rc = _timed_optional("dle_gemm", C.lib().dle_gemm_expand_masked_bnred2,
                          (C.ptr(g2), C.ptr(w), C.ptr(out), C.ptr(addend), C.ptr(bits), C.ptr(t2), C.ptr(bits2), C.ptr(mean2),
                           C.ptr(rstd2), C.ptr(ws), ws.numel() * 4, m, n, k, g2.stride(0), w.stride(0), out.stride(0), 0, C.dt(g2),
                           C.stream()))
     if rc > 1:
-        C.check(rc - 1000 if rc > 1000 else -1, "dle_gemm_expand_masked_bnred")
+        C.check(rc - 1000 if rc > 1000 else -1, "dle_gemm_expand_masked_bnred2")
     if rc != 1:
         return None
     C.call("dle_bn_bwd_finish", C.ptr(ws), groups, n, C.ptr(dgamma2), C.ptr(dbeta2), 0, C.stream())
diff --git a/include/dle_mi355x.h b/include/dle_mi355x.h
--- a/include/dle_mi355x.h
+++ b/include/dle_mi355x.h
@@ -237,6 +237,9 @@
 int dle_gemm_expand_masked_bnred(const void* A, const void* B, void* C, const void* src, const void* bits, const void* t2,
                                  const void* bits2, const float* mean2, const float* rstd2, float* partial, int64_t partial_bytes,
                                  int M, int N, int K, int64_t lda, int64_t ldb, int64_t ldc, int b_kc, int dtype, hipStream_t stream);
+int dle_gemm_expand_masked_bnred2(const void* A, const void* B, void* C, const void* src, const void* bits, const void* t2,
+                                  const void* bits2, const float* mean2, const float* rstd2, float* partial, int64_t partial_bytes,
+                                  int M, int N, int K, int64_t lda, int64_t ldb, int64_t ldc, int b_kc, int dtype, hipStream_t stream);
 int dle_bn_bwd_finish(const float* partial, int groups, int C, float* dgamma, float* dbeta, int accumulate, hipStream_t stream);
 int dle_stem_conv7_groups(int N, int H);
 int dle_stem_conv7_fwd(const void* x4, const void* w2, void* y, float* stats, int64_t stats_bytes, int N, int H, int W,
@@ -259,6 +262,10 @@
 int dle_avgpool_bwd(const void* dy, void* dx, int64_t N, int HW, int C, int dtype, hipStream_t stream);
 int dle_gemm_expand_add_up2(const void* A, const void* B, void* C, const void* compact, int M, int N, int K, int64_t lda,
                             int64_t ldb, int64_t ldc, int64_t ld_compact, int b_kc, int H, int W, int dtype, hipStream_t stream);
+int dle_gemm_expand_add_up2_bnred(const void* A, const void* B, void* C, const void* compact, const void* t2, const void* bits2,
+                                  const float* mean2, const float* rstd2, float* partial, int64_t partial_bytes, int M, int N, int K,
+                                  int64_t lda, int64_t ldb, int64_t ldc, int64_t ld_compact, int b_kc, int H, int W, int dtype,
+                                  hipStream_t stream);
 int dle_upsample_zero(const void* x, void* y, int64_t N, int P, int Q, int H, int W, int C, int stride, int dtype,
                       hipStream_t stream);
 int dle_softmax_xent(const float* logits, const int64_t* target, float* loss_out, void* dlogits,
```

New measurement: 13530 samples/s, median of 6. Within noise of the previous version (+0.7%).
